# AIRI-Institute/nablaDFT

Measured on NVIDIA H100. Metric: molecules/sec (PaiNN E+F fwd+bwd), higher is better.
Workload: dtype f32

## Files before the change

include/nabla_b200.h:

```cpp
#ifndef NABLA_B200_H
#define NABLA_B200_H

#include <stdint.h>

#ifdef __cplusplus
extern "C" {
#endif

#define NB200_OK 0
#define NB200_EINVAL -1
#define NB200_EUNSUPPORTED -2
#define NB200_ECUDA -3
#define NB200_ECAPACITY -4
#define NB200_ENEIGHBORS -5
#define NB200_ENOEDGES -6

#define NB200_RADIAL_SPK 0
#define NB200_RADIAL_OC 1

int nb200_version(void);
int nb200_last_cuda_error(void);

int nb200_neighbor_build(const float* pos, const int32_t* mol_ptr, int32_t n_mol, int32_t n_atoms,
                         float cutoff, int32_t max_neighbors, int32_t e_cap,
                         int32_t* row_ptr, int32_t* col, int32_t* rev, float* geom,
                         int32_t* deg_scratch, int32_t* status, void* stream);

int nb200_painn_filter(const float* geom, const int32_t* status, int32_t e_stride,
                       const float* w_rbf, const float* b_rbf, int32_t n_layers, int32_t n_rbf,
                       int32_t n_feat, int32_t radial_mode, float cutoff,
                       const float* rbf_offsets, float rbf_coeff, float rbf_xscale,
                       float* W, float* dW, int32_t* sort_scratch, void* stream);

int nb200_painn_msg_fwd(const float* xh, const float* xh_bias, const float* q, const float* mu,
                        const float* W, const float* geom, const int32_t* row_ptr,
                        const int32_t* col, int32_t n_atoms, float* q_out, float* mu_out,
                        void* stream);

int nb200_painn_msg_bwd(const float* xh, const float* xh_bias, const float* mu,
                        const float* W, const float* dW, const float* geom,
                        const int32_t* row_ptr, const int32_t* col, int32_t n_atoms,
                        const float* g_q, const float* g_mu,
                        float* g_xh, float* g_mu_in, float* egrad, void* stream);

int nb200_painn_msg_fwd_ex(const float* xh, const float* xh_bias, const float* q, const float* mu,
                           const void* W, int32_t w_stride, const int32_t* rev, const float* geom,
                           const int32_t* row_ptr, const int32_t* col, int32_t n_atoms, float* q_out,
                           float* mu_out, int32_t bf16, void* stream);
int nb200_painn_msg_bwd_ex(const float* xh, const float* xh_bias, const float* mu, const void* W,
                           const void* dW, int32_t w_stride, const int32_t* rev, const float* geom,
                           const int32_t* row_ptr, const int32_t* col, int32_t n_atoms, const float* g_q,
                           const float* g_mu, float* g_xh, float* g_mu_in, float* egrad, void* gW,
                           const float* seed_atom, int32_t bf16, void* stream);
int nb200_msg_gather_probe(const float* A, const float* B, const float* rec, int32_t rec_stride,
                           const int32_t* rev, const int32_t* row_ptr, const int32_t* col, int32_t n_atoms,
                           int32_t bwd_pattern, float* out, void* stream);

int nb200_edge_forces(const float* egrad, const float* geom, const int32_t* row_ptr,
                      const int32_t* rev, int32_t n_atoms, float* forces, void* stream);

typedef struct nb200_painn_weights {
    int32_t n_layers, n_feat, n_rbf, n_elem;
    int32_t radial_mode, z_offset;
    float cutoff, epsilon;
    float rbf_coeff, rbf_xscale;
    const float* rbf_offsets;
    float energy_shift_per_atom;
    int32_t max_neighbors;
    const float* emb;
    const float* w_rbf;
    const float* b_rbf;
    const float* A1; const float* c1;
    const float* A2; const float* c2;
    const float* U;
    const float* B1; const float* d1;
    const float* B2; const float* d2;
    const float* R1; const float* e1;
    const float* R2; const float* e2;
} nb200_painn_weights;

typedef struct nb200_engine nb200_engine;

int nb200_engine_create(nb200_engine** out);
int nb200_engine_destroy(nb200_engine* eng);
int nb200_engine_set_timing(nb200_engine* eng, int32_t enable);
int nb200_engine_read_timings(nb200_engine* eng, float* ms_per_cat, int32_t* scopes_per_cat, int32_t n_cat);
int nb200_engine_set_gemm_backend(nb200_engine* eng, int32_t backend);
int nb200_engine_set_node_backend(nb200_engine* eng, int32_t backend);
int nb200_gemm_tf32x3(int32_t M, int32_t N, int32_t K, const float* A, int32_t lda, const float* B,
                      int32_t ldb, int32_t trans_b, float* C, int32_t ldc, int32_t accumulate,
                      const float* bias, float* act, void* stream);
int nb200_linear_wgrad(int32_t M, int32_t out, int32_t in, const float* G0, const float* X0, const float* G1,
                       const float* X1, int32_t ldg, int32_t ldx, float* dW, int32_t lddw, float alpha,
                       float* dbias, float bias_alpha, const float* row_scale, int32_t rs_div, void* stream);
int nb200_engine_set_edge_storage(nb200_engine* eng, int32_t bf16);
int64_t nb200_engine_own_launches(nb200_engine* eng);
int64_t nb200_painn_workspace_bytes(const nb200_painn_weights* w, int32_t b_cap, int32_t n_cap,
                                    int32_t e_cap, int32_t with_forces);
int nb200_painn_energy_forces(nb200_engine* eng, const nb200_painn_weights* w,
                              const int32_t* z, const float* pos, const int32_t* mol_ptr,
                              int32_t n_mol, int32_t n_atoms, int32_t e_cap,
                              void* workspace, int64_t workspace_bytes,
                              float* energy, float* forces, int32_t* status, void* stream);
int64_t nb200_painn_train_workspace_bytes(const nb200_painn_weights* w, int32_t b_cap, int32_t n_cap,
                                          int32_t e_cap, int32_t with_force_seed);
int nb200_painn_energy_forces_grads(nb200_engine* eng, const nb200_painn_weights* w,
                                    const int32_t* z, const float* pos, const int32_t* mol_ptr,
                                    int32_t n_mol, int32_t n_atoms, int32_t e_cap,
                                    void* workspace, int64_t workspace_bytes,
                                    const float* energy_seed, const float* force_seed,
                                    const nb200_painn_weights* grads,
                                    float* energy, float* forces, int32_t* status, void* stream);
int nb200_painn_train_forward(nb200_engine* eng, const nb200_painn_weights* w,
                              const int32_t* z, const float* pos, const int32_t* mol_ptr,
                              int32_t n_mol, int32_t n_atoms, int32_t e_cap,
                              void* workspace, int64_t workspace_bytes, int32_t with_force_seed,
                              float* energy, float* forces, int32_t* status, void* stream);
int nb200_painn_train_backward(nb200_engine* eng, const nb200_painn_weights* w,
                               const int32_t* z, const int32_t* mol_ptr,
                               int32_t n_mol, int32_t n_atoms, int32_t e_cap,
                               void* workspace, int64_t workspace_bytes, int32_t with_force_seed,
                               const float* energy_seed, const float* force_seed,
                               const nb200_painn_weights* grads, int32_t* status, void* stream);
int64_t nb200_painn_hvp_workspace_bytes(const nb200_painn_weights* w, int32_t b_cap, int32_t n_cap, int32_t e_cap, int32_t n_dir);
int nb200_painn_hvp(nb200_engine* eng, const nb200_painn_weights* w, const int32_t* z, const float* pos, const int32_t* mol_ptr,
                    int32_t n_mol, int32_t n_atoms, int32_t e_cap, void* workspace, int64_t workspace_bytes,
                    int32_t n_dir, const float* v, float* energy, float* forces, float* hv, int32_t* status, void* stream);

typedef struct nb200_schnet_weights {
    int32_t n_layers, n_feat, n_rbf, n_elem;
    int32_t z_offset;
    float cutoff, rbf_coeff;
    float energy_shift_per_atom;
    const float* rbf_offsets;
    const float* emb;
    const float* w_f1; const float* b_f1;
    const float* W_f2; const float* b_f2;
    const float* I1;
    const float* P1; const float* p1;
    const float* P2; const float* p2;
    const float* R1; const float* e1;
    const float* R2; const float* e2;
} nb200_schnet_weights;

int64_t nb200_schnet_workspace_bytes(const nb200_schnet_weights* w, int32_t b_cap, int32_t n_cap,
                                     int32_t e_cap, int32_t with_forces);
int nb200_schnet_energy_forces(nb200_engine* eng, const nb200_schnet_weights* w,
                               const int32_t* z, const float* pos, const int32_t* mol_ptr,
                               int32_t n_mol, int32_t n_atoms, int32_t e_cap,
                               void* workspace, int64_t workspace_bytes,
                               float* energy, float* forces, int32_t* status, void* stream);

int nb200_schnet_train_count(const nb200_schnet_weights* w, const float* pos, const int32_t* mol_ptr, int32_t n_mol, int32_t n_atoms,
                             int32_t* row_ptr, int32_t* scratch, int64_t* n_edges_host, void* stream);
int64_t nb200_schnet_train_workspace_bytes(const nb200_schnet_weights* w, int32_t n_mol, int32_t n_atoms, int64_t n_edges,
                                           int32_t with_force_seed);
int nb200_schnet_energy_grads(nb200_engine* eng, const nb200_schnet_weights* w, const int32_t* z, const float* pos, const int32_t* mol_ptr,
                              int32_t n_mol, int32_t n_atoms, const int32_t* row_ptr, int64_t n_edges, void* workspace,
                              int64_t workspace_bytes, const float* energy_seed, const float* force_seed,
                              const nb200_schnet_weights* grads, float* energy, void* stream);
int64_t nb200_schnet_hvp_workspace_bytes(const nb200_schnet_weights* w, int32_t n_mol, int32_t n_atoms, int64_t n_edges);
int nb200_schnet_hvp(nb200_engine* eng, const nb200_schnet_weights* w, const int32_t* z, const float* pos, const int32_t* mol_ptr,
                     int32_t n_mol, int32_t n_atoms, const int32_t* row_ptr, int64_t n_edges, void* workspace, int64_t workspace_bytes,
                     int32_t n_dir, const float* v, float* energy, float* forces, float* hv, void* stream);

int nb200_qh_expand_rows(const int32_t* row_ptr, int32_t n_atoms, int32_t* tgt, void* stream);
int nb200_qh_edge_basis(const float* geom, const int32_t* status, int32_t e_cap, double alpha, float cutoff,
                        float sign, const double* logc, int32_t n_rbf, float* rbf, float* sh, void* stream);
int nb200_qh_norm_feats(const float* x, int32_t n_rows, float* f0, void* stream);
int nb200_qh_gate(const float* x, const float* gates, int32_t n_rows, float* y, void* stream);
int nb200_qh_invariants(const float* f, const int32_t* tgt, const int32_t* col, const int32_t* status,
                        int32_t e_cap, int32_t mode, float* out, void* stream);
int nb200_qh_tp_conv(const float* x, const float* sh, const float* w1, const float* w2, const int32_t* row_ptr,
                     const int32_t* col, int32_t n_atoms, int32_t layer0, int32_t add_self, float* out, void* stream);
int nb200_qh_tp_pair(const float* x, const float* w1, const float* w2, const int32_t* tgt, const int32_t* col,
                     const int32_t* status, int32_t p_cap, float* out, void* stream);
int nb200_qh_tp_self(const float* xl, const float* xr, const float* w, const float* res, int32_t n_rows,
                     float* out, void* stream);
int nb200_qh_linear(const float* x, const float* W_l, const float* bias, int32_t n_rows, int32_t c_in,
                    int32_t c_out, int32_t accumulate, float* y, void* stream);
int nb200_dense(int32_t M, int32_t N, int32_t K, const float* A, int32_t lda, const float* B, int32_t ldb,
                int32_t trans_b, float* C, int32_t ldc, int32_t accumulate, const float* bias, float* act,
                int32_t act_kind, void* stream);
int nb200_qh_expand_setup(const int32_t* ins_host, const float* cg_host);
int nb200_qh_expand(const float* x, const float* W, const float* Bw, int32_t bw_stride, int32_t n_rows,
                    float* blocks, void* stream);
int nb200_qh_pair_hidden(const float* A, const float* Bn, const float* bias, const int32_t* tgt,
                         const int32_t* col, const int32_t* status, int32_t p_cap, float* h, void* stream);
int nb200_qh_assemble(const float* diag, const float* offd, const int32_t* z, const int32_t* tgt,
                      const int32_t* col, const int32_t* rev, int32_t n_atoms, int32_t n_pairs,
                      const int32_t* mask_tab, const int32_t* norb_tab, const int32_t* atom_mol,
                      const int32_t* atom_orb_off, const int64_t* mol_h_off, const int32_t* mol_norb,
                      float* H, void* stream);
int nb200_axpy(float* y, const float* x, int64_t n, void* stream);

int64_t nb200_lbfgs_state_bytes(int32_t n_mol, int32_t n_atoms, int32_t memory);
int nb200_lbfgs_step(void* state, int64_t state_bytes, const int32_t* mol_ptr, int32_t n_mol, int32_t n_atoms,
                     int32_t max_atoms_per_mol, int32_t memory, int32_t iteration, double fmax, double maxstep,
                     double damping, double h0, const uint8_t* fixed_mask, double* pos, float* forces,
                     float* pos32_out, int32_t* unconverged_out, int32_t* n_normalizations, void* stream);

int nb200_md_init_momenta(const int32_t* mol_ptr, int32_t n_mol, const double* mass, const double* pos, double kT, uint64_t seed,
                          int64_t noise_step, double* mom, void* stream);
int nb200_md_step(const int32_t* mol_ptr, int32_t n_mol, const double* mass, int32_t phase, int32_t thermostat, double dt, double kT,
                  double gamma, uint64_t seed, int64_t step, double f_scale, double e_scale, double* pos, double* mom, float* pos32,
                  const float* forces, const float* energy, double* log_slot, double* frame_pos, double* frame_mom,
                  const int32_t* status, int32_t* worst, void* stream);

enum {
    NB200_GOC_G_RBF_OFFSET = 0,
    NB200_GOC_G_EMB,
    NB200_GOC_G_CAT_MAIN,
    NB200_GOC_G_CAT_AE,
    NB200_GOC_G_CAT_Q,
    NB200_GOC_G_CAT_A2A,
    NB200_GOC_G_EDGE_EMB,
    NB200_GOC_G_OUT_E0,
    NB200_GOC_G_OUT_E_RES,
    NB200_GOC_G_OUT_ENERGY,
    NB200_GOC_G_OUT_F0,
    NB200_GOC_G_OUT_F_RES,
    NB200_GOC_G_OUT_FORCES,
    NB200_GOC_G_COUNT
};
enum {
    NB200_GOC_I_DENSE_CA = 0,
    NB200_GOC_I_T_BA, NB200_GOC_I_T_RBF , NB200_GOC_I_T_BIL , NB200_GOC_I_T_DOWN ,
    NB200_GOC_I_T_UPCA , NB200_GOC_I_T_UPAC,
    NB200_GOC_I_Q_DB, NB200_GOC_I_Q_RBF, NB200_GOC_I_Q_CBF , NB200_GOC_I_Q_BIL , NB200_GOC_I_Q_DOWN ,
    NB200_GOC_I_Q_UPCA , NB200_GOC_I_Q_UPAC,
    NB200_GOC_I_AE_BA , NB200_GOC_I_AE_RBF , NB200_GOC_I_AE_BIL, NB200_GOC_I_AE_DOWN ,
    NB200_GOC_I_AE_UPCA , NB200_GOC_I_AE_UPAC,
    NB200_GOC_I_EA_BA , NB200_GOC_I_EA_RBF, NB200_GOC_I_EA_BIL, NB200_GOC_I_EA_DOWN , NB200_GOC_I_EA_UP ,
    NB200_GOC_I_AA_BIL , NB200_GOC_I_AA_DOWN , NB200_GOC_I_AA_UP ,
    NB200_GOC_I_BEFORE_SKIP,
    NB200_GOC_I_AFTER_SKIP,
    NB200_GOC_I_AU_RBF , NB200_GOC_I_AU_L0 , NB200_GOC_I_AU_RES ,
    NB200_GOC_I_CONCAT , NB200_GOC_I_RES_M ,
    NB200_GOC_I_COUNT
};
enum {
    NB200_GOC_O_RBF = 0 , NB200_GOC_O_L0 , NB200_GOC_O_RES ,
    NB200_GOC_O_E2 , NB200_GOC_O_F , NB200_GOC_O_RBF_F ,
    NB200_GOC_O_COUNT
};
enum {
    NB200_GOC_S_T_RBF = 0, NB200_GOC_S_Q_RBF, NB200_GOC_S_Q_CBF, NB200_GOC_S_AE_RBF, NB200_GOC_S_EA_RBF, NB200_GOC_S_AU_SUM, NB200_GOC_S_COUNT
};
enum { NB200_GOC_SO_SUM = 0, NB200_GOC_SO_RBF_F, NB200_GOC_SO_COUNT };
enum {
    NB200_GOC_C_A2A = 0,
    NB200_GOC_C_MAIN,
    NB200_GOC_C_AE,
    NB200_GOC_C_Q,
    NB200_GOC_C_TIN,
    NB200_GOC_C_COUNT = 8
};
typedef struct nb200_gemnet_oc_weights {
    int32_t num_blocks;
    int32_t n_elem;
    float cutoff;
    int32_t max_neighbors, max_neighbors_qint, max_neighbors_aeaint;
    const float* w;
    const int64_t* off_host;
    const float* scale_host;
} nb200_gemnet_oc_weights;
int64_t nb200_gemnet_oc_graph_bytes(int32_t n_atoms, int32_t max_atoms_per_mol);
int nb200_gemnet_oc_graph_count(const nb200_gemnet_oc_weights* w, const float* pos, const int32_t* mol_ptr, int32_t n_mol,
                                int32_t n_atoms, int32_t max_atoms_per_mol, void* graph_buf, int64_t graph_bytes,
                                int64_t* counts_host, void* stream);
int64_t nb200_gemnet_oc_workspace_bytes(const nb200_gemnet_oc_weights* w, int32_t n_mol, int32_t n_atoms, const int64_t* counts_host);
int nb200_gemnet_oc_energy_forces(nb200_engine* eng, const nb200_gemnet_oc_weights* w, const int32_t* z, const float* pos,
                                  const int32_t* mol_ptr, int32_t n_mol, int32_t n_atoms, int32_t max_atoms_per_mol,
                                  void* graph_buf, int64_t graph_bytes, const int64_t* counts_host, void* workspace,
                                  int64_t workspace_bytes, float* energy, float* forces, void* stream);
int nb200_gemnet_oc_count_bounds(const nb200_gemnet_oc_weights* w, const int32_t* mol_ptr_host, int32_t n_mol, int64_t* counts_bound_host);
int nb200_gemnet_oc_energy_forces_async(nb200_engine* eng, const nb200_gemnet_oc_weights* w, const int32_t* z, const float* pos,
                                        const int32_t* mol_ptr, int32_t n_mol, int32_t n_atoms, int32_t max_atoms_per_mol,
                                        void* graph_buf, int64_t graph_bytes, const int64_t* counts_bound_host, void* workspace,
                                        int64_t workspace_bytes, float* energy, float* forces, int32_t* status, void* stream);
int64_t nb200_gemnet_oc_train_workspace_bytes(const nb200_gemnet_oc_weights* w, int32_t n_mol, int32_t n_atoms, const int64_t* counts_host);
int nb200_gemnet_oc_energy_forces_grads(nb200_engine* eng, const nb200_gemnet_oc_weights* w, int64_t n_weights, const int32_t* z,
                                        const float* pos, const int32_t* mol_ptr, int32_t n_mol, int32_t n_atoms, int32_t max_atoms_per_mol,
                                        void* graph_buf, int64_t graph_bytes, const int64_t* counts_host, void* workspace,
                                        int64_t workspace_bytes, const float* energy_seed, const float* force_seed, float* grads,
                                        float* energy, float* forces, int64_t* keep_token_host, void* stream);
int nb200_gemnet_oc_backward(nb200_engine* eng, int64_t token, const float* energy_seed, const float* force_seed, void* stream);
int nb200_gemnet_oc_debug_h(const void* workspace, const nb200_gemnet_oc_weights* w, int32_t n_mol, int32_t n_atoms,
                            const int64_t* counts_host, float* h_out, void* stream);

enum {
    NB200_DPP_G_FREQ = 0,
    NB200_DPP_G_ZEROS,
    NB200_DPP_G_NORMS,
    NB200_DPP_G_EMB_TI,
    NB200_DPP_G_EMB_TJ,
    NB200_DPP_G_EMB_RBF_W,
    NB200_DPP_G_EMB_RBF_B,
    NB200_DPP_G_EMB_W3,
    NB200_DPP_G_HEAD_W0, NB200_DPP_G_HEAD_B0,
    NB200_DPP_G_HEAD_W1, NB200_DPP_G_HEAD_B1,
    NB200_DPP_G_HEAD_W2, NB200_DPP_G_HEAD_B2,
    NB200_DPP_G_HEAD_W3, NB200_DPP_G_HEAD_B3,
    NB200_DPP_G_COUNT
};
enum {
    NB200_DPP_I_RBF = 0,
    NB200_DPP_I_SBF,
    NB200_DPP_I_SBF1,
    NB200_DPP_I_SBF2,
    NB200_DPP_I_JI_W, NB200_DPP_I_JI_B, NB200_DPP_I_KJ_W, NB200_DPP_I_KJ_B,
    NB200_DPP_I_DOWN,
    NB200_DPP_I_UP,
    NB200_DPP_I_RES_W,
    NB200_DPP_I_RES_B,
    NB200_DPP_I_LIN_W, NB200_DPP_I_LIN_B,
    NB200_DPP_I_COUNT
};
enum {
    NB200_DPP_O_RBF = 0,
    NB200_DPP_O_UP,
    NB200_DPP_O_LINS_W,
    NB200_DPP_O_LINS_B,
    NB200_DPP_O_LIN,
    NB200_DPP_O_COUNT
};
enum { NB200_DPP_C_EDGES = 0, NB200_DPP_C_TRIPLETS, NB200_DPP_C_COUNT = 4 };
typedef struct nb200_dimenet_weights {
    int32_t num_blocks, node_latent_dim, hidden, int_emb, basis_emb, out_emb, num_spherical, num_radial;
    int32_t num_before_skip, num_after_skip, num_output_layers, envelope_exponent, max_neighbors;
    float cutoff, scale, mean;
    const float* w;
    const int64_t* off_host;
} nb200_dimenet_weights;
int64_t nb200_dimenet_graph_bytes(const nb200_dimenet_weights* w, int32_t n_atoms);
int nb200_dimenet_graph_count(const nb200_dimenet_weights* w, const int32_t* z, const float* pos, const int32_t* mol_ptr, int32_t n_mol,
                              int32_t n_atoms, void* graph_buf, int64_t graph_bytes, int64_t* counts_host, void* stream);
int64_t nb200_dimenet_workspace_bytes(const nb200_dimenet_weights* w, int32_t n_mol, int32_t n_atoms, const int64_t* counts_host);
int nb200_dimenet_energy_forces(nb200_engine* eng, const nb200_dimenet_weights* w, const int32_t* z, const float* pos, const int32_t* mol_ptr,
                                int32_t n_mol, int32_t n_atoms, void* graph_buf, int64_t graph_bytes, const int64_t* counts_host,
                                void* workspace, int64_t workspace_bytes, float* energy, float* forces, float* graph_emb, void* stream);
int nb200_dimenet_debug_sbf_radial(const nb200_dimenet_weights* w, const float* dist, int32_t n, float* rbs, float* drbs, void* stream);

int nb200_phis_n_paths(int32_t order_in1, int32_t order_in2, int32_t order_out, int32_t strict_upper);
int nb200_phis_pair_mixing(const float* x1, const float* x2, const float* coeff, int32_t n_rows, int32_t n_feat,
                           int32_t order_in1, int32_t order_in2, int32_t order_out, float* y, void* stream);
int nb200_phis_self_mixing(const float* x, const float* mixcoeff, const float* keepcoeff, int32_t n_rows, int32_t n_feat,
                           int32_t order_in, int32_t order_out, float* y, void* stream);
int nb200_phis_linear(const float* x, const float* W_l, const float* bias, int32_t n_rows, int32_t c_in, int32_t c_out,
                      int32_t order, float* y, void* stream);

int nb200_phis_swish_self_mixing(const float* x, const float* alpha, const float* beta, const float* mixcoeff, const float* keepcoeff,
                                 int32_t n_rows, int32_t n_feat, float* y, void* stream);
int nb200_phis_linear_ex(const float* x, const float* W_l, const float* bias, int32_t n_rows, int32_t c_in, int32_t c_out, int32_t order,
                         int32_t accumulate, float* y, void* stream);
int nb200_phis_interaction(const float* yi, const float* yj, const float* sh, const float* coeff, const float* wa1, const float* ba1,
                           const float* wa2, const float* ba2, const int32_t* row_ptr, const int32_t* col, int32_t n_atoms, int32_t n_feat,
                           float* y, void* stream);
int nb200_phis_pair_features(const float* fpc, const float* fpn, const float* coeff, const int32_t* row_ptr, const int32_t* col,
                             int32_t n_atoms, int32_t n_feat, float* fii, float* fij, void* stream);
int nb200_phis_overlap_pairs(const float* x, const float* sh, const float* coeff, const float* wa, const int32_t* row_ptr,
                             const int32_t* col, int32_t n_atoms, int32_t n_feat, float* s, void* stream);
int nb200_phis_assemble(const float* Xd, const float* Xo, const float* Wd, const float* bd, int32_t n_col_d, const float* Wo, const float* bo,
                        int32_t n_col_o, int32_t n_feat, const int32_t* atom_el, const int32_t* row_orb, const int32_t* row_m,
                        const int32_t* orb_l, const int32_t* n_rows, const int32_t* ent_range, const int32_t* op_base, const int32_t* ent_col,
                        const int32_t* ent_L, int32_t n_el, int32_t max_ent, const int32_t* tgt, const int32_t* col, const int32_t* rev,
                        int32_t n_atoms, int32_t n_pairs, const int32_t* atom_mol, const int32_t* atom_off, const int64_t* mol_off,
                        const int32_t* mol_norb, int32_t unit_diagonal, float* M, void* stream);

#ifdef __cplusplus
}
#endif
#endif
```

nabladft_b200/_lib.py:

```python
import ctypes
import os
from ctypes import c_double, POINTER, c_float, c_int32, c_int64, c_uint64, c_void_p

_HERE = os.path.dirname(os.path.abspath(__file__))
LIB_PATH = os.path.join(_HERE, "libnabla_b200.so")

NB200_OK = 0
ERRORS = {
    -1: "NB200_EINVAL (bad argument)",
    -2: "NB200_EUNSUPPORTED (configuration outside the compiled fast path)",
    -3: "NB200_ECUDA (CUDA runtime / cuBLAS error)",
    -4: "NB200_ECAPACITY (edge capacity exceeded)",
    -5: "NB200_ENEIGHBORS (an atom has more than max_neighbors neighbours)",
    -6: "NB200_ENOEDGES (an atom has no neighbours)",
}
RADIAL_SPK, RADIAL_OC = 0, 1

_fp = POINTER(c_float)


class PainnWeights(ctypes.Structure):

    _fields_ = [
        ("n_layers", c_int32), ("n_feat", c_int32), ("n_rbf", c_int32), ("n_elem", c_int32),
        ("radial_mode", c_int32), ("z_offset", c_int32),
        ("cutoff", c_float), ("epsilon", c_float),
        ("rbf_coeff", c_float), ("rbf_xscale", c_float),
        ("rbf_offsets", c_void_p),
        ("energy_shift_per_atom", c_float),
        ("max_neighbors", c_int32),
        ("emb", c_void_p), ("w_rbf", c_void_p), ("b_rbf", c_void_p),
        ("A1", c_void_p), ("c1", c_void_p), ("A2", c_void_p), ("c2", c_void_p),
        ("U", c_void_p),
        ("B1", c_void_p), ("d1", c_void_p), ("B2", c_void_p), ("d2", c_void_p),
        ("R1", c_void_p), ("e1", c_void_p), ("R2", c_void_p), ("e2", c_void_p),
    ]


class SchnetWeights(ctypes.Structure):

    _fields_ = [
        ("n_layers", c_int32), ("n_feat", c_int32), ("n_rbf", c_int32), ("n_elem", c_int32),
        ("z_offset", c_int32),
        ("cutoff", c_float), ("rbf_coeff", c_float),
        ("energy_shift_per_atom", c_float),
        ("rbf_offsets", c_void_p),
        ("emb", c_void_p),
        ("w_f1", c_void_p), ("b_f1", c_void_p), ("W_f2", c_void_p), ("b_f2", c_void_p),
        ("I1", c_void_p),
        ("P1", c_void_p), ("p1", c_void_p), ("P2", c_void_p), ("p2", c_void_p),
        ("R1", c_void_p), ("e1", c_void_p), ("R2", c_void_p), ("e2", c_void_p),
    ]


class GemNetOCWeights(ctypes.Structure):

    _fields_ = [("num_blocks", c_int32), ("n_elem", c_int32), ("cutoff", c_float), ("max_neighbors", c_int32), ("max_neighbors_qint", c_int32),
                ("max_neighbors_aeaint", c_int32), ("w", c_void_p), ("off_host", POINTER(c_int64)), ("scale_host", POINTER(c_float))]


class DimeNetWeights(ctypes.Structure):

    _fields_ = [("num_blocks", c_int32), ("node_latent_dim", c_int32), ("hidden", c_int32), ("int_emb", c_int32), ("basis_emb", c_int32),
                ("out_emb", c_int32), ("num_spherical", c_int32), ("num_radial", c_int32), ("num_before_skip", c_int32), ("num_after_skip", c_int32),
                ("num_output_layers", c_int32), ("envelope_exponent", c_int32), ("max_neighbors", c_int32), ("cutoff", c_float), ("scale", c_float),
                ("mean", c_float), ("w", c_void_p), ("off_host", POINTER(c_int64))]


SIGNATURES = {
    "nb200_version": (c_int32, []),
    "nb200_last_cuda_error": (c_int32, []),
    "nb200_neighbor_build": (c_int32, [c_void_p, c_void_p, c_int32, c_int32, c_float, c_int32, c_int32,
                                       c_void_p, c_void_p, c_void_p, c_void_p, c_void_p, c_void_p, c_void_p]),
    "nb200_painn_filter": (c_int32, [c_void_p, c_void_p, c_int32, c_void_p, c_void_p, c_int32, c_int32, c_int32, c_int32,
                                     c_float, c_void_p, c_float, c_float, c_void_p, c_void_p, c_void_p, c_void_p]),
    "nb200_painn_msg_fwd": (c_int32, [c_void_p] * 8 + [c_int32, c_void_p, c_void_p, c_void_p]),
    "nb200_painn_msg_bwd": (c_int32, [c_void_p] * 8 + [c_int32] + [c_void_p] * 6),
    "nb200_edge_forces": (c_int32, [c_void_p, c_void_p, c_void_p, c_void_p, c_int32, c_void_p, c_void_p]),
    "nb200_painn_msg_fwd_ex": (c_int32, [c_void_p] * 5 + [c_int32] + [c_void_p] * 4 + [c_int32] + [c_void_p] * 2 + [c_int32, c_void_p]),
    "nb200_painn_msg_bwd_ex": (c_int32, [c_void_p] * 5 + [c_int32] + [c_void_p] * 4 + [c_int32] + [c_void_p] * 7 + [c_int32, c_void_p]),
    "nb200_msg_gather_probe": (c_int32, [c_void_p] * 3 + [c_int32] + [c_void_p] * 3 + [c_int32, c_int32, c_void_p, c_void_p]),
    "nb200_engine_create": (c_int32, [POINTER(c_void_p)]),
    "nb200_engine_destroy": (c_int32, [c_void_p]),
    "nb200_engine_set_timing": (c_int32, [c_void_p, c_int32]),
    "nb200_engine_read_timings": (c_int32, [c_void_p, c_void_p, c_void_p, c_int32]),
    "nb200_engine_own_launches": (c_int64, [c_void_p]),
    "nb200_engine_set_gemm_backend": (c_int32, [c_void_p, c_int32]),
    "nb200_engine_set_node_backend": (c_int32, [c_void_p, c_int32]),
    "nb200_phis_n_paths": (c_int32, [c_int32, c_int32, c_int32, c_int32]),
    "nb200_phis_pair_mixing": (c_int32, [c_void_p, c_void_p, c_void_p, c_int32, c_int32, c_int32, c_int32, c_int32, c_void_p, c_void_p]),
    "nb200_phis_self_mixing": (c_int32, [c_void_p, c_void_p, c_void_p, c_int32, c_int32, c_int32, c_int32, c_void_p, c_void_p]),
    "nb200_phis_linear": (c_int32, [c_void_p, c_void_p, c_void_p, c_int32, c_int32, c_int32, c_int32, c_void_p, c_void_p]),
    "nb200_phis_swish_self_mixing": (c_int32, [c_void_p] * 5 + [c_int32, c_int32, c_void_p, c_void_p]),
    "nb200_phis_linear_ex": (c_int32, [c_void_p, c_void_p, c_void_p, c_int32, c_int32, c_int32, c_int32, c_int32, c_void_p, c_void_p]),
    "nb200_phis_interaction": (c_int32, [c_void_p] * 10 + [c_int32, c_int32, c_void_p, c_void_p]),
    "nb200_phis_pair_features": (c_int32, [c_void_p] * 5 + [c_int32, c_int32, c_void_p, c_void_p, c_void_p]),
    "nb200_phis_overlap_pairs": (c_int32, [c_void_p] * 6 + [c_int32, c_int32, c_void_p, c_void_p]),
    "nb200_phis_assemble": (c_int32, [c_void_p] * 4 + [c_int32] + [c_void_p] * 2 + [c_int32, c_int32] + [c_void_p] * 9 + [c_int32, c_int32]
                            + [c_void_p] * 3 + [c_int32, c_int32] + [c_void_p] * 4 + [c_int32, c_void_p, c_void_p]),
    "nb200_gemm_tf32x3": (c_int32, [c_int32, c_int32, c_int32, c_void_p, c_int32, c_void_p, c_int32, c_int32, c_void_p, c_int32,
                                    c_int32, c_void_p, c_void_p, c_void_p]),
    "nb200_linear_wgrad": (c_int32, [c_int32, c_int32, c_int32, c_void_p, c_void_p, c_void_p, c_void_p, c_int32, c_int32, c_void_p, c_int32, c_float,
                                     c_void_p, c_float, c_void_p, c_int32, c_void_p]),
    "nb200_qh_expand_rows": (c_int32, [c_void_p, c_int32, c_void_p, c_void_p]),
    "nb200_qh_edge_basis": (c_int32, [c_void_p, c_void_p, c_int32, c_double, c_float, c_float, c_void_p, c_int32, c_void_p, c_void_p, c_void_p]),
    "nb200_qh_norm_feats": (c_int32, [c_void_p, c_int32, c_void_p, c_void_p]),
    "nb200_qh_gate": (c_int32, [c_void_p, c_void_p, c_int32, c_void_p, c_void_p]),
    "nb200_qh_invariants": (c_int32, [c_void_p, c_void_p, c_void_p, c_void_p, c_int32, c_int32, c_void_p, c_void_p]),
    "nb200_qh_tp_conv": (c_int32, [c_void_p] * 6 + [c_int32, c_int32, c_int32, c_void_p, c_void_p]),
    "nb200_qh_tp_pair": (c_int32, [c_void_p] * 6 + [c_int32, c_void_p, c_void_p]),
    "nb200_qh_tp_self": (c_int32, [c_void_p] * 4 + [c_int32, c_void_p, c_void_p]),
    "nb200_qh_linear": (c_int32, [c_void_p, c_void_p, c_void_p, c_int32, c_int32, c_int32, c_int32, c_void_p, c_void_p]),
    "nb200_dense": (c_int32, [c_int32, c_int32, c_int32, c_void_p, c_int32, c_void_p, c_int32, c_int32, c_void_p, c_int32, c_int32,
                              c_void_p, c_void_p, c_int32, c_void_p]),
    "nb200_qh_expand_setup": (c_int32, [c_void_p, c_void_p]),
    "nb200_qh_expand": (c_int32, [c_void_p, c_void_p, c_void_p, c_int32, c_int32, c_void_p, c_void_p]),
    "nb200_qh_pair_hidden": (c_int32, [c_void_p] * 6 + [c_int32, c_void_p, c_void_p]),
    "nb200_qh_assemble": (c_int32, [c_void_p] * 6 + [c_int32, c_int32] + [c_void_p] * 8),
    "nb200_axpy": (c_int32, [c_void_p, c_void_p, c_int64, c_void_p]),
    "nb200_lbfgs_state_bytes": (c_int64, [c_int32, c_int32, c_int32]),
    "nb200_lbfgs_step": (c_int32, [c_void_p, c_int64, c_void_p, c_int32, c_int32, c_int32, c_int32, c_int32, c_double, c_double, c_double,
                                   c_double, c_void_p, c_void_p, c_void_p, c_void_p, c_void_p, c_void_p, c_void_p]),
    "nb200_md_init_momenta": (c_int32, [c_void_p, c_int32, c_void_p, c_void_p, c_double, c_uint64, c_int64, c_void_p, c_void_p]),
    "nb200_md_step": (c_int32, [c_void_p, c_int32, c_void_p, c_int32, c_int32, c_double, c_double, c_double, c_uint64, c_int64, c_double, c_double]
                      + [c_void_p] * 11),
    "nb200_painn_workspace_bytes": (c_int64, [POINTER(PainnWeights), c_int32, c_int32, c_int32, c_int32]),
    "nb200_schnet_workspace_bytes": (c_int64, [POINTER(SchnetWeights), c_int32, c_int32, c_int32, c_int32]),
    "nb200_schnet_energy_forces": (c_int32, [c_void_p, POINTER(SchnetWeights), c_void_p, c_void_p, c_void_p, c_int32, c_int32,
                                             c_int32, c_void_p, c_int64, c_void_p, c_void_p, c_void_p, c_void_p]),
    "nb200_painn_train_workspace_bytes": (c_int64, [POINTER(PainnWeights), c_int32, c_int32, c_int32, c_int32]),
    "nb200_painn_energy_forces_grads": (c_int32, [c_void_p, POINTER(PainnWeights), c_void_p, c_void_p, c_void_p, c_int32, c_int32, c_int32,
                                                  c_void_p, c_int64, c_void_p, c_void_p, POINTER(PainnWeights), c_void_p, c_void_p, c_void_p,
                                                  c_void_p]),
    "nb200_engine_set_edge_storage": (c_int32, [c_void_p, c_int32]),
    "nb200_painn_train_forward": (c_int32, [c_void_p, POINTER(PainnWeights), c_void_p, c_void_p, c_void_p, c_int32, c_int32, c_int32,
                                            c_void_p, c_int64, c_int32, c_void_p, c_void_p, c_void_p, c_void_p]),
    "nb200_painn_train_backward": (c_int32, [c_void_p, POINTER(PainnWeights), c_void_p, c_void_p, c_int32, c_int32, c_int32,
                                             c_void_p, c_int64, c_int32, c_void_p, c_void_p, POINTER(PainnWeights), c_void_p, c_void_p]),
    "nb200_painn_energy_forces": (c_int32, [c_void_p, POINTER(PainnWeights), c_void_p, c_void_p, c_void_p, c_int32, c_int32,
                                            c_int32, c_void_p, c_int64, c_void_p, c_void_p, c_void_p, c_void_p]),
    "nb200_painn_hvp_workspace_bytes": (c_int64, [POINTER(PainnWeights), c_int32, c_int32, c_int32, c_int32]),
    "nb200_painn_hvp": (c_int32, [c_void_p, POINTER(PainnWeights), c_void_p, c_void_p, c_void_p, c_int32, c_int32, c_int32, c_void_p, c_int64,
                                  c_int32, c_void_p, c_void_p, c_void_p, c_void_p, c_void_p, c_void_p]),

    "nb200_gemnet_oc_graph_bytes": (c_int64, [c_int32, c_int32]),
    "nb200_gemnet_oc_graph_count": (c_int32, [POINTER(GemNetOCWeights), c_void_p, c_void_p, c_int32, c_int32, c_int32, c_void_p, c_int64,
                                              POINTER(c_int64), c_void_p]),
    "nb200_gemnet_oc_workspace_bytes": (c_int64, [POINTER(GemNetOCWeights), c_int32, c_int32, POINTER(c_int64)]),
    "nb200_gemnet_oc_energy_forces": (c_int32, [c_void_p, POINTER(GemNetOCWeights), c_void_p, c_void_p, c_void_p, c_int32, c_int32, c_int32,
                                                c_void_p, c_int64, POINTER(c_int64), c_void_p, c_int64, c_void_p, c_void_p, c_void_p]),
    "nb200_gemnet_oc_count_bounds": (c_int32, [POINTER(GemNetOCWeights), POINTER(c_int32), c_int32, POINTER(c_int64)]),
    "nb200_gemnet_oc_energy_forces_async": (c_int32, [c_void_p, POINTER(GemNetOCWeights), c_void_p, c_void_p, c_void_p, c_int32, c_int32, c_int32,
                                                      c_void_p, c_int64, POINTER(c_int64), c_void_p, c_int64, c_void_p, c_void_p, c_void_p, c_void_p]),
    "nb200_gemnet_oc_debug_h": (c_int32, [c_void_p, POINTER(GemNetOCWeights), c_int32, c_int32, POINTER(c_int64), c_void_p, c_void_p]),
    "nb200_schnet_train_count": (c_int32, [POINTER(SchnetWeights), c_void_p, c_void_p, c_int32, c_int32, c_void_p, c_void_p, POINTER(c_int64), c_void_p]),
    "nb200_schnet_train_workspace_bytes": (c_int64, [POINTER(SchnetWeights), c_int32, c_int32, c_int64, c_int32]),
    "nb200_schnet_energy_grads": (c_int32, [c_void_p, POINTER(SchnetWeights), c_void_p, c_void_p, c_void_p, c_int32, c_int32, c_void_p, c_int64, c_void_p,
                                            c_int64, c_void_p, c_void_p, POINTER(SchnetWeights), c_void_p, c_void_p]),
    "nb200_schnet_hvp_workspace_bytes": (c_int64, [POINTER(SchnetWeights), c_int32, c_int32, c_int64]),
    "nb200_schnet_hvp": (c_int32, [c_void_p, POINTER(SchnetWeights), c_void_p, c_void_p, c_void_p, c_int32, c_int32, c_void_p, c_int64, c_void_p,
                                   c_int64, c_int32, c_void_p, c_void_p, c_void_p, c_void_p, c_void_p]),
    "nb200_gemnet_oc_train_workspace_bytes": (c_int64, [POINTER(GemNetOCWeights), c_int32, c_int32, POINTER(c_int64)]),
    "nb200_gemnet_oc_energy_forces_grads": (c_int32, [c_void_p, POINTER(GemNetOCWeights), c_int64, c_void_p, c_void_p, c_void_p, c_int32, c_int32, c_int32,
                                                      c_void_p, c_int64, POINTER(c_int64), c_void_p, c_int64, c_void_p, c_void_p, c_void_p, c_void_p, c_void_p,
                                                      POINTER(c_int64), c_void_p]),
    "nb200_gemnet_oc_backward": (c_int32, [c_void_p, c_int64, c_void_p, c_void_p, c_void_p]),
    "nb200_dimenet_graph_bytes": (c_int64, [POINTER(DimeNetWeights), c_int32]),
    "nb200_dimenet_graph_count": (c_int32, [POINTER(DimeNetWeights), c_void_p, c_void_p, c_void_p, c_int32, c_int32, c_void_p, c_int64,
                                            POINTER(c_int64), c_void_p]),
    "nb200_dimenet_workspace_bytes": (c_int64, [POINTER(DimeNetWeights), c_int32, c_int32, POINTER(c_int64)]),
    "nb200_dimenet_energy_forces": (c_int32, [c_void_p, POINTER(DimeNetWeights), c_void_p, c_void_p, c_void_p, c_int32, c_int32, c_void_p, c_int64,
                                              POINTER(c_int64), c_void_p, c_int64, c_void_p, c_void_p, c_void_p, c_void_p]),
    "nb200_dimenet_debug_sbf_radial": (c_int32, [POINTER(DimeNetWeights), c_void_p, c_int32, c_void_p, c_void_p, c_void_p]),
}

_lib = None


class NablaB200Error(RuntimeError):
    pass


def load():
    global _lib
    if _lib is not None:
        return _lib
    if not os.path.exists(LIB_PATH):
        raise NablaB200Error(
            f"{LIB_PATH} is missing: build it with `python -m nabladft_b200.build` "
            "(nvcc, sm_90a). There is no CPU / eager fallback for this path."
        )
    lib = ctypes.CDLL(LIB_PATH)
    for name, (res, args) in SIGNATURES.items():
        fn = getattr(lib, name)
        fn.restype, fn.argtypes = res, args
    _lib = lib
    return lib


def check(rc: int, what: str):
    if rc != NB200_OK:
        detail = ERRORS.get(rc, f"error {rc}")
        cuda = load().nb200_last_cuda_error() if rc == -3 else 0
        raise NablaB200Error(f"{what} failed: {detail}" + (f" [cudaError {cuda}]" if cuda else ""))


def ptr(t):
    if t is None:
        return None
    assert t.is_contiguous(), "C ABI takes contiguous buffers"
    return c_void_p(t.data_ptr())


def current_stream():
    import torch

    return c_void_p(torch.cuda.current_stream().cuda_stream)
```

nabladft_b200/csrc/painn_fused.cu:

```cuda
#include "painn_node.cuh"

#include "tc_pipe.cuh"

namespace {

constexpr int TILES_PER_LAYER = 22;

enum { T_UV = 0, T_UW, T_B1A, T_B1B, T_B2_0, T_B2_1, T_B2_2, T_A1, T_A2_0, T_A2_1, T_A2_2,
       T_B2T_0, T_B2T_1, T_B2T_2, T_B1AT, T_B1BT, T_UT_0, T_UT_1, T_A2T_0, T_A2T_1, T_A2T_2, T_A1T };

struct TileSrc { const float* p; int ld, row0, k0, trans, rows, kvalid; };

__device__ __forceinline__ TileSrc tile_src(const nb200_painn_weights& w, int idx) {
    const int L = w.n_layers;
    TileSrc s{nullptr, F, 0, 0, 0, 128, 128};
    if (idx >= L * TILES_PER_LAYER) {
        s.p = w.R1; s.ld = F;
        if (idx - L * TILES_PER_LAYER == 0) { s.rows = F / 2; } else { s.trans = 1; s.kvalid = F / 2; }
        return s;
    }
    const int l = idx / TILES_PER_LAYER, t = idx % TILES_PER_LAYER;
    const float* A1 = w.A1 + (size_t)l * F * F;
    const float* A2 = w.A2 + (size_t)l * 3 * F * F;
    const float* U = w.U + (size_t)l * 2 * F * F;
    const float* B1 = w.B1 + (size_t)l * F * 2 * F;
    const float* B2 = w.B2 + (size_t)l * 3 * F * F;
    switch (t) {
        case T_UV: s.p = U; break;
        case T_UW: s.p = U; s.row0 = F; break;
        case T_B1A: s.p = B1; s.ld = 2 * F; break;
        case T_B1B: s.p = B1; s.ld = 2 * F; s.k0 = F; break;
        case T_B2_0: case T_B2_1: case T_B2_2: s.p = B2; s.row0 = (t - T_B2_0) * F; break;
        case T_A1: s.p = A1; break;
        case T_A2_0: case T_A2_1: case T_A2_2: s.p = A2; s.row0 = (t - T_A2_0) * F; break;
        case T_B2T_0: case T_B2T_1: case T_B2T_2: s.p = B2; s.trans = 1; s.k0 = (t - T_B2T_0) * F; break;
        case T_B1AT: s.p = B1; s.ld = 2 * F; s.trans = 1; break;
        case T_B1BT: s.p = B1; s.ld = 2 * F; s.trans = 1; s.row0 = F; break;
        case T_UT_0: case T_UT_1: s.p = U; s.trans = 1; s.k0 = (t - T_UT_0) * F; break;
        case T_A2T_0: case T_A2T_1: case T_A2T_2: s.p = A2; s.trans = 1; s.k0 = (t - T_A2T_0) * F; break;
        default: s.p = A1; s.trans = 1; break;
    }
    return s;
}

__global__ void __launch_bounds__(256) k_prep_painn(nb200_painn_weights w, unsigned char* __restrict__ dst) {
    const int idx = blockIdx.x >> 2, st = blockIdx.x & 3;
    const TileSrc s = tile_src(w, idx);
    unsigned char* tile = dst + (size_t)idx * WTILE_BYTES;
#pragma unroll
    for (int i = 0; i < 4; ++i) {
        const int item = threadIdx.x + 256 * i;
        int kc, r;
        if (!s.trans) { kc = item & 7; r = item >> 3; } else { r = item & 127; kc = item >> 7; }
        const int k = st * 32 + kc * 4;
        float e[4];
#pragma unroll
        for (int j = 0; j < 4; ++j) {
            const bool ok = r < s.rows && k + j < s.kvalid;
            e[j] = !ok ? 0.f : !s.trans ? __ldg(s.p + (size_t)(s.row0 + r) * s.ld + s.k0 + k + j) : __ldg(s.p + (size_t)(s.k0 + k + j) * s.ld + s.row0 + r);
        }
        float4 hi, lo;
        split4(make_float4(e[0], e[1], e[2], e[3]), hi, lo);
        const int kk = 32 * st + 4 * kc;
        float* out_hi = reinterpret_cast<float*>(tile + (size_t)(kk / KSTAGE) * WST_BYTES + (size_t)((kk % KSTAGE) / 4) * WLBO) + r * 4;
        st4(out_hi, hi);
        st4(out_hi + (KSTAGE / 4) * WLBO / 4, lo);
    }
}

struct FwdParams {
    int n_atoms, do_upd, do_mlp, do_ro;
    const unsigned char* wt;
    int tile_upd, tile_mlp, tile_ro;
    const float *q_mid, *mu_mid, *d1, *d2;
    float *VW, *nrm, *dot, *g1pre, *y, *q_next, *mu_next;
    float eps;
    const float *q_mlp_in, *c1;
    float *h1pre, *xh;
    float* ro_pre;
};

template <class L>
__global__ void __launch_bounds__(NTHREADS, CTAS_PER_SM) k_node_fwd(const FwdParams P) {
    constexpr int CW = L::CW;
    extern __shared__ __align__(1024) unsigned char smem[];
    __shared__ Prog prog;
    const int tid = threadIdx.x, warp = tid >> 5, lane = tid & 31;
    if (tid == 0) {
        prog.n = 0;
        if (P.do_upd) {
            for (int x = 0; x < 3; ++x) {
                prog_add(prog, P.tile_upd + T_UV, U_NEWX | U_FIRST | U_LAST);
                prog_add(prog, P.tile_upd + T_UW, U_FIRST | U_LAST | U_XLAST);
            }
            prog_add(prog, P.tile_upd + T_B1A, U_NEWX | U_FIRST | U_LAST | U_XLAST);
            prog_add(prog, P.tile_upd + T_B1B, U_NEWX | U_FIRST | U_LAST | U_XLAST);
            prog_add(prog, P.tile_upd + T_B2_1, U_NEWX | U_FIRST | U_LAST);
            prog_add(prog, P.tile_upd + T_B2_0, U_FIRST | U_LAST);
            prog_add(prog, P.tile_upd + T_B2_2, U_FIRST | U_LAST | U_XLAST);
        }
        if (P.do_mlp) {
            prog_add(prog, P.tile_mlp + T_A1, U_NEWX | U_FIRST | U_LAST | U_XLAST);
            prog_add(prog, P.tile_mlp + T_A2_0, U_NEWX | U_FIRST | U_LAST);
            prog_add(prog, P.tile_mlp + T_A2_1, U_FIRST | U_LAST);
            prog_add(prog, P.tile_mlp + T_A2_2, U_FIRST | U_LAST | U_XLAST);
        }
        if (P.do_ro) prog_add(prog, P.tile_ro, U_NEWX | U_FIRST | U_LAST | U_XLAST);
    }
    Ctx<L> c = setup<L>(smem, tid);

    if (warp >= WARP_ISSUE) {
        role_regs<L>(true);
        run_issuer(c, prog, P.wt);
    } else {
        role_regs<L>(false);
        const int N = P.n_atoms, A0 = blockIdx.x * L::NT;
        const int fl = 32 * (warp & 3) + lane;
        const int n0 = L::CPT * (warp >> 2);
        if (P.do_upd) {
#pragma unroll 1
            for (int x = 0; x < 3; ++x) {
                load_x(c, tid, [&](int r, int kc) { return A0 + r < N ? ldg4(P.mu_mid + (size_t)(A0 + r) * (3 * F) + x * F + 4 * kc) : f4(0.f); });
#pragma unroll 1
                for (int half = 0; half < 2; ++half) {
                    drain(c, warp);
                    epi_chunks(c, warp, [&](int cb, float (&v)[CW]) {
                        float* dst = P.VW + (size_t)(A0 + n0 + CW * cb) * (6 * F) + x * 2 * F + half * F + fl;
#pragma unroll
                        for (int j = 0; j < CW; ++j)
                            if (A0 + n0 + CW * cb + j < N) dst[(size_t)j * (6 * F)] = v[j];
                    });
                }
            }
            work_barrier();
            load_x(c, tid, [&](int r, int kc) { return A0 + r < N ? ldg4(P.q_mid + (size_t)(A0 + r) * F + 4 * kc) : f4(0.f); });
            {
                const int kc = tid & 31, w = tid >> 5;
#pragma unroll 1
                for (int it0 = 0; it0 < L::RPT; it0 += 2) {
                    float4 V[2][3], Wv[2][3];
#pragma unroll
                    for (int b = 0; b < 2; ++b) {
                        const int a = A0 + w + L::NLOAD * (it0 + b);
                        const float* vv = P.VW + (size_t)min(a, N - 1) * (6 * F) + 4 * kc;
#pragma unroll
                        for (int x = 0; x < 3; ++x) { V[b][x] = ld4(vv + x * 2 * F); Wv[b][x] = ld4(vv + x * 2 * F + F); }
                    }
#pragma unroll
                    for (int b = 0; b < 2; ++b) {
                        const int a = A0 + w + L::NLOAD * (it0 + b);
                        if (a < N) {
                            float4 sq = V[b][0] * V[b][0]; fma4(sq, V[b][1], V[b][1]); fma4(sq, V[b][2], V[b][2]);
                            float4 dt = f4(0.f); fma4(dt, V[b][0], Wv[b][0]); fma4(dt, V[b][1], Wv[b][1]); fma4(dt, V[b][2], Wv[b][2]);
                            st4(P.nrm + (size_t)a * F + 4 * kc, make_float4(sqrtf(sq.x + P.eps), sqrtf(sq.y + P.eps), sqrtf(sq.z + P.eps), sqrtf(sq.w + P.eps)));
                            st4(P.dot + (size_t)a * F + 4 * kc, dt);
                        }
                    }
                }
            }
            work_barrier();
            load_x(c, tid, [&](int r, int kc) { return A0 + r < N ? ld4(P.nrm + (size_t)(A0 + r) * F + 4 * kc) : f4(0.f); });
            drain(c, warp);
            {
                drain(c, warp, 1);
                const float b = __ldg(P.d1 + fl);
                const XPut xp(c, fl);
                epi_chunks(c, warp, [&](int cb, float (&v)[CW]) {
#pragma unroll
                    for (int j = 0; j < CW; ++j) xp.put(n0 + CW * cb + j, A0 + n0 + CW * cb + j < N ? siluf_(v[j] + b) : 0.f);
                });
                xp.done(c);
                epi_chunks(c, warp, [&](int cb, float (&v)[CW]) {
                    float* g = P.g1pre + (size_t)(A0 + n0 + CW * cb) * F + fl;
#pragma unroll
                    for (int j = 0; j < CW; ++j)
                        if (A0 + n0 + CW * cb + j < N) g[(size_t)j * F] = v[j] + b;
                });
            }
            {
                drain(c, warp);
                const float b = __ldg(P.d2 + F + fl);
#pragma unroll 1
                for (int cb = 0; cb < L::CPT / 8; ++cb) {
                    float v8[8];
                    stage_ld(c, warp, 8 * cb, v8);
                    float tw[8][3], tm[8][3];
#pragma unroll
                    for (int jj = 0; jj < 8; ++jj) {
                        const int a = min(A0 + n0 + 8 * cb + jj, N - 1);
                        const float* vw = P.VW + (size_t)a * (6 * F) + F + fl;
                        const float* mm = P.mu_mid + (size_t)a * (3 * F) + fl;
#pragma unroll
                        for (int x = 0; x < 3; ++x) { tw[jj][x] = vw[x * 2 * F]; tm[jj][x] = __ldg(mm + x * F); }
                    }
#pragma unroll
                    for (int jj = 0; jj < 8; ++jj) {
                        const int a = A0 + n0 + 8 * cb + jj;
                        if (a < N) {
                            const float y1 = v8[jj] + b;
                            P.y[(size_t)a * (3 * F) + F + fl] = y1;
                            float* mo = P.mu_next + (size_t)a * (3 * F) + fl;
#pragma unroll
                            for (int x = 0; x < 3; ++x) mo[x * F] = fmaf(y1, tw[jj][x], tm[jj][x]);
                        }
                    }
                }
            }
            {
                drain(c, warp);
                const float b = __ldg(P.d2 + fl);
                epi_chunks(c, warp, [&](int cb, float (&v)[CW]) {
                    float t[CW];
#pragma unroll
                    for (int j = 0; j < CW; ++j) t[j] = __ldg(P.q_mid + (size_t)min(A0 + n0 + CW * cb + j, N - 1) * F + fl);
#pragma unroll
                    for (int j = 0; j < CW; ++j) {
                        const int a = A0 + n0 + CW * cb + j;
                        if (a < N) {
                            const float y0 = v[j] + b;
                            P.y[(size_t)a * (3 * F) + fl] = y0;
                            P.q_next[(size_t)a * F + fl] = t[j] + y0;
                        }
                    }
                });
            }
            {
                drain(c, warp);
                const float b = __ldg(P.d2 + 2 * F + fl);
                const XPut xp(c, fl);
                epi_chunks(c, warp, [&](int cb, float (&v)[CW]) {
                    float tq[CW], td[CW];
#pragma unroll
                    for (int j = 0; j < CW; ++j) {
                        const size_t a = (size_t)min(A0 + n0 + CW * cb + j, N - 1);
                        tq[j] = P.q_next[a * F + fl];
                        td[j] = P.dot[a * F + fl];
                    }
#pragma unroll
                    for (int j = 0; j < CW; ++j) {
                        const int a = A0 + n0 + CW * cb + j;
                        float qn = 0.f;
                        if (a < N) {
                            qn = fmaf(v[j] + b, td[j], tq[j]);
                            P.q_next[(size_t)a * F + fl] = qn;
                        }
                        xp.put(n0 + CW * cb + j, qn);
                    }
                });
                xp.done(c);
                epi_chunks(c, warp, [&](int cb, float (&v)[CW]) {
#pragma unroll
                    for (int j = 0; j < CW; ++j)
                        if (A0 + n0 + CW * cb + j < N) P.y[(size_t)(A0 + n0 + CW * cb + j) * (3 * F) + 2 * F + fl] = v[j] + b;
                });
            }
        } else {
            load_x(c, tid, [&](int r, int kc) { return A0 + r < N ? ldg4(P.q_mlp_in + (size_t)(A0 + r) * F + 4 * kc) : f4(0.f); });
        }
        if (P.do_mlp) {
            {
                drain(c, warp);
                const float b = __ldg(P.c1 + fl);
                const XPut xp(c, fl);
                epi_chunks(c, warp, [&](int cb, float (&v)[CW]) {
#pragma unroll
                    for (int j = 0; j < CW; ++j) xp.put(n0 + CW * cb + j, siluf_(v[j] + b));
                });
                xp.done(c);
                epi_chunks(c, warp, [&](int cb, float (&v)[CW]) {
#pragma unroll
                    for (int j = 0; j < CW; ++j)
                        if (A0 + n0 + CW * cb + j < N) P.h1pre[(size_t)(A0 + n0 + CW * cb + j) * F + fl] = v[j] + b;
                });
            }
#pragma unroll 1
            for (int ct = 0; ct < 3; ++ct) {
                drain(c, warp);
                epi_chunks(c, warp, [&](int cb, float (&v)[CW]) {
                    float* dst = P.xh + (size_t)(A0 + n0 + CW * cb) * (3 * F) + ct * F + fl;
#pragma unroll
                    for (int j = 0; j < CW; ++j)
                        if (A0 + n0 + CW * cb + j < N) dst[(size_t)j * (3 * F)] = v[j];
                });
            }
        }
        if (P.do_ro) {
            drain(c, warp);
            epi_chunks(c, warp, [&](int cb, float (&v)[CW]) {
                if (fl < F / 2) {
                    float* dst = P.ro_pre + (size_t)(A0 + n0 + CW * cb) * (F / 2) + fl;
#pragma unroll
                    for (int j = 0; j < CW; ++j)
                        if (A0 + n0 + CW * cb + j < N) dst[(size_t)j * (F / 2)] = v[j];
                }
            });
        }
    }
}

struct BwdParams {
    int n_atoms, do_mlp, do_ro, do_upd;
    const unsigned char* wt;
    int tile_mlp, tile_ro, tile_upd;
    float *gq_a, *gq_b, *cur, *gn, *gdot;
    const float *g_xh, *h1pre, *dot;
    const float *ro_pre, *R2;
    const float *y, *VW, *nrm, *g1pre;
};

template <class L>
__global__ void __launch_bounds__(NTHREADS, CTAS_PER_SM) k_node_bwd(const BwdParams P) {
    constexpr int CW = L::CW;
    extern __shared__ __align__(1024) unsigned char smem[];
    __shared__ Prog prog;
    const int tid = threadIdx.x, warp = tid >> 5, lane = tid & 31;
    if (tid == 0) {
        prog.n = 0;
        if (P.do_mlp) {
            prog_add(prog, P.tile_mlp + T_A2T_0, U_NEWX | U_FIRST | U_XLAST);
            prog_add(prog, P.tile_mlp + T_A2T_1, U_NEWX | U_XLAST);
            prog_add(prog, P.tile_mlp + T_A2T_2, U_NEWX | U_XLAST | U_LAST);
            prog_add(prog, P.tile_mlp + T_A1T, U_NEWX | U_FIRST | U_LAST | U_XLAST);
        } else if (P.do_ro) {
            prog_add(prog, P.tile_ro, U_NEWX | U_FIRST | U_LAST | U_XLAST);
        }
        if (P.do_upd) {
            prog_add(prog, P.tile_upd + T_B2T_0, U_NEWX | U_FIRST | U_XLAST);
            prog_add(prog, P.tile_upd + T_B2T_1, U_NEWX | U_XLAST);
            prog_add(prog, P.tile_upd + T_B2T_2, U_NEWX | U_XLAST | U_LAST);
            prog_add(prog, P.tile_upd + T_B1AT, U_NEWX | U_FIRST | U_LAST);
            prog_add(prog, P.tile_upd + T_B1BT, U_FIRST | U_LAST | U_XLAST);
            for (int x = 0; x < 3; ++x) {
                prog_add(prog, P.tile_upd + T_UT_0, U_NEWX | U_FIRST | U_XLAST);
                prog_add(prog, P.tile_upd + T_UT_1, U_NEWX | U_XLAST | U_LAST);
            }
        }
    }
    Ctx<L> c = setup<L>(smem, tid);

    if (warp >= WARP_ISSUE) {
        role_regs<L>(true);
        run_issuer(c, prog, P.wt);
    } else {
        role_regs<L>(false);
        const int N = P.n_atoms, A0 = blockIdx.x * L::NT;
        const int fl = 32 * (warp & 3) + lane;
        const int n0 = L::CPT * (warp >> 2);
        if (P.do_mlp) {
#pragma unroll 1
            for (int ck = 0; ck < 3; ++ck)
                load_x(c, tid, [&](int r, int kc) { return A0 + r < N ? ldg4(P.g_xh + (size_t)(A0 + r) * (3 * F) + ck * F + 4 * kc) : f4(0.f); });
            drain(c, warp);
            const XPut xp(c, fl);
            epi_chunks(c, warp, [&](int cb, float (&v)[CW]) {
                float t[CW];
#pragma unroll
                for (int j = 0; j < CW; ++j) t[j] = __ldg(P.h1pre + (size_t)min(A0 + n0 + CW * cb + j, N - 1) * F + fl);
#pragma unroll
                for (int j = 0; j < CW; ++j) xp.put(n0 + CW * cb + j, A0 + n0 + CW * cb + j < N ? v[j] * dsiluf_(t[j]) : 0.f);
            });
            xp.done(c);
        } else if (P.do_ro) {
            load_x(c, tid, [&](int r, int kc) {
                if (A0 + r >= N || kc >= F / 8) return f4(0.f);
                const float4 p = ldg4(P.ro_pre + (size_t)(A0 + r) * (F / 2) + 4 * kc), w2 = ldg4(P.R2 + 4 * kc);
                return make_float4(w2.x * dsiluf_(p.x), w2.y * dsiluf_(p.y), w2.z * dsiluf_(p.z), w2.w * dsiluf_(p.w));
            });
        }
        if (P.do_mlp || P.do_ro) {
            drain(c, warp);
            epi_chunks(c, warp, [&](int cb, float (&v)[CW]) {
                float t[CW], ty[CW];
#pragma unroll
                for (int j = 0; j < CW; ++j) {
                    const size_t a = (size_t)min(A0 + n0 + CW * cb + j, N - 1);
                    t[j] = P.do_mlp ? P.gq_a[a * F + fl] : 0.f;
                    ty[j] = P.do_upd ? __ldg(P.y + a * (3 * F) + 2 * F + fl) : 0.f;
                }
#pragma unroll
                for (int j = 0; j < CW; ++j) {
                    const int a = A0 + n0 + CW * cb + j;
                    if (a < N) {
                        const float g = t[j] + v[j];
                        P.gq_b[(size_t)a * F + fl] = g;
                        if (P.do_upd) P.gdot[(size_t)a * F + fl] = g * ty[j];
                    }
                }
            });
        }
        if (P.do_upd) {
            work_barrier();
            load_x(c, tid, [&](int r, int kc) { return A0 + r < N ? ld4(P.gq_b + (size_t)(A0 + r) * F + 4 * kc) : f4(0.f); });
            load_x(c, tid, [&](int r, int kc) {
                if (A0 + r >= N) return f4(0.f);
                const float* vw = P.VW + (size_t)(A0 + r) * (6 * F) + F + 4 * kc;
                const float* gm = P.cur + (size_t)(A0 + r) * (3 * F) + 4 * kc;
                float4 sacc = f4(0.f);
#pragma unroll
                for (int x = 0; x < 3; ++x) fma4(sacc, ld4(gm + x * F), ldg4(vw + x * 2 * F));
                return sacc;
            });
            load_x(c, tid, [&](int r, int kc) {
                return A0 + r < N ? ld4(P.gq_b + (size_t)(A0 + r) * F + 4 * kc) * ldg4(P.dot + (size_t)(A0 + r) * F + 4 * kc) : f4(0.f);
            });
            drain(c, warp);
            const XPut xp(c, fl);
            epi_chunks(c, warp, [&](int cb, float (&v)[CW]) {
                float t[CW];
#pragma unroll
                for (int j = 0; j < CW; ++j) t[j] = __ldg(P.g1pre + (size_t)min(A0 + n0 + CW * cb + j, N - 1) * F + fl);
#pragma unroll
                for (int j = 0; j < CW; ++j) xp.put(n0 + CW * cb + j, A0 + n0 + CW * cb + j < N ? v[j] * dsiluf_(t[j]) : 0.f);
            });
            xp.done(c);
            {
                drain(c, warp);
                epi_chunks(c, warp, [&](int cb, float (&v)[CW]) {
                    float t[CW];
#pragma unroll
                    for (int j = 0; j < CW; ++j) t[j] = P.gq_b[(size_t)min(A0 + n0 + CW * cb + j, N - 1) * F + fl];
#pragma unroll
                    for (int j = 0; j < CW; ++j)
                        if (A0 + n0 + CW * cb + j < N) P.gq_a[(size_t)(A0 + n0 + CW * cb + j) * F + fl] = t[j] + v[j];
                });
            }
            {
                drain(c, warp);
                epi_chunks(c, warp, [&](int cb, float (&v)[CW]) {
                    float t[CW];
#pragma unroll
                    for (int j = 0; j < CW; ++j) t[j] = __ldg(P.nrm + (size_t)min(A0 + n0 + CW * cb + j, N - 1) * F + fl);
#pragma unroll
                    for (int j = 0; j < CW; ++j)
                        if (A0 + n0 + CW * cb + j < N) P.gn[(size_t)(A0 + n0 + CW * cb + j) * F + fl] = v[j] / t[j];
                });
            }
            work_barrier();
#pragma unroll 1
            for (int x = 0; x < 3; ++x) {
                load_x(c, tid, [&](int r, int kc) {
                    if (A0 + r >= N) return f4(0.f);
                    const size_t a = (size_t)(A0 + r);
                    float4 o = ld4(P.gdot + a * F + 4 * kc) * ldg4(P.VW + a * (6 * F) + x * 2 * F + F + 4 * kc);
                    fma4(o, ld4(P.gn + a * F + 4 * kc), ldg4(P.VW + a * (6 * F) + x * 2 * F + 4 * kc));
                    return o;
                });
                load_x(c, tid, [&](int r, int kc) {
                    if (A0 + r >= N) return f4(0.f);
                    const size_t a = (size_t)(A0 + r);
                    float4 o = ld4(P.cur + a * (3 * F) + x * F + 4 * kc) * ldg4(P.y + a * (3 * F) + F + 4 * kc);
                    fma4(o, ld4(P.gdot + a * F + 4 * kc), ldg4(P.VW + a * (6 * F) + x * 2 * F + 4 * kc));
                    return o;
                });
                drain(c, warp);
                epi_chunks(c, warp, [&](int cb, float (&v)[CW]) {
                    float t[CW];
#pragma unroll
                    for (int j = 0; j < CW; ++j) t[j] = P.cur[(size_t)min(A0 + n0 + CW * cb + j, N - 1) * (3 * F) + x * F + fl];
#pragma unroll
                    for (int j = 0; j < CW; ++j)
                        if (A0 + n0 + CW * cb + j < N) P.cur[(size_t)(A0 + n0 + CW * cb + j) * (3 * F) + x * F + fl] = t[j] + v[j];
                });
            }
        }
    }
}

using Node64 = Layout<false, 64>;
using Node80 = Layout<false, 80>;

bool wide_tiles(int n_atoms) {
    const int sm = nb_sm_count();
    const int waves64 = ((n_atoms + Node64::NT - 1) / Node64::NT + sm - 1) / sm, waves80 = ((n_atoms + Node80::NT - 1) / Node80::NT + sm - 1) / sm;
    return waves80 < waves64;
}

template <class L, class Params>
int launch_tiles(void (*kernel)(Params), const Params& P, int n_atoms, cudaStream_t s) {
    static std::atomic<bool> attr[NB_MAX_DEVICES];
    int dev = 0;
    cudaGetDevice(&dev);
    const bool cached = dev >= 0 && dev < NB_MAX_DEVICES;
    if (!cached || !attr[dev].load(std::memory_order_relaxed)) {
        if (cudaFuncSetAttribute(kernel, cudaFuncAttributeMaxDynamicSharedMemorySize, L::SMEM_TOTAL) != cudaSuccess) { nb_check_launch(); return NB200_ECUDA; }
        if (cached) attr[dev].store(true, std::memory_order_relaxed);
    }
    kernel<<<(n_atoms + L::NT - 1) / L::NT, NTHREADS, L::SMEM_TOTAL, s>>>(P);
    return nb_check_launch();
}

}

int64_t nb_fused_wtile_bytes(int n_layers) { return (int64_t)(n_layers * TILES_PER_LAYER + 2) * WTILE_BYTES; }

int nb_fused_prep(const nb200_painn_weights* w, void* wtiles, cudaStream_t s) {
    const int n_tiles = w->n_layers * TILES_PER_LAYER + 2;
    k_prep_painn<<<n_tiles * 4, 256, 0, s>>>(*w, static_cast<unsigned char*>(wtiles));
    return nb_check_launch();
}

int nb_fused_node_fwd(const NbFusedFwd& a, cudaStream_t s) {
    FwdParams P{};
    P.n_atoms = a.n_atoms; P.do_upd = a.layer_upd >= 0; P.do_mlp = a.layer_mlp >= 0; P.do_ro = a.readout;
    P.wt = static_cast<const unsigned char*>(a.wtiles);
    P.tile_upd = a.layer_upd * TILES_PER_LAYER; P.tile_mlp = a.layer_mlp * TILES_PER_LAYER; P.tile_ro = a.n_layers * TILES_PER_LAYER;
    P.q_mid = a.q_mid; P.mu_mid = a.mu_mid; P.d1 = a.d1; P.d2 = a.d2; P.VW = a.VW; P.nrm = a.nrm; P.dot = a.dot; P.g1pre = a.g1pre; P.y = a.y;
    P.q_next = a.q_next; P.mu_next = a.mu_next; P.eps = a.eps; P.q_mlp_in = a.q_mlp_in; P.c1 = a.c1; P.h1pre = a.h1pre; P.xh = a.xh;
    P.ro_pre = a.ro_pre;
    if (a.n_atoms <= 0) return NB200_OK;
    return wide_tiles(a.n_atoms) ? launch_tiles<Node80>(k_node_fwd<Node80>, P, a.n_atoms, s) : launch_tiles<Node64>(k_node_fwd<Node64>, P, a.n_atoms, s);
}

int nb_fused_node_bwd(const NbFusedBwd& a, cudaStream_t s) {
    BwdParams P{};
    P.n_atoms = a.n_atoms; P.do_mlp = a.layer_mlp >= 0; P.do_ro = a.readout; P.do_upd = a.layer_upd >= 0;
    P.wt = static_cast<const unsigned char*>(a.wtiles);
    P.tile_mlp = a.layer_mlp * TILES_PER_LAYER; P.tile_ro = a.n_layers * TILES_PER_LAYER + 1; P.tile_upd = a.layer_upd * TILES_PER_LAYER;
    P.gq_a = a.gq_a; P.gq_b = a.gq_b; P.cur = a.cur; P.gn = a.gn; P.gdot = a.gdot; P.dot = a.dot; P.g_xh = a.g_xh; P.h1pre = a.h1pre; P.ro_pre = a.ro_pre; P.R2 = a.R2;
    P.y = a.y; P.VW = a.VW; P.nrm = a.nrm; P.g1pre = a.g1pre;
    if (a.n_atoms <= 0) return NB200_OK;
    return wide_tiles(a.n_atoms) ? launch_tiles<Node80>(k_node_bwd<Node80>, P, a.n_atoms, s) : launch_tiles<Node64>(k_node_bwd<Node64>, P, a.n_atoms, s);
}
```

nabladft_b200/csrc/tc_pipe.cuh:

```cuda
#pragma once
#include "common.cuh"
#include "wgmma.cuh"

namespace {


constexpr int F = NB_F;
constexpr int KSTAGE = 32, W_STAGES = 3, NWORK = 8, CTAS_PER_SM = 1;
constexpr int WLBO = 128 * 16;
constexpr int WST_BYTES = 2 * (KSTAGE / 4) * WLBO;
constexpr int STAGES_PER_TILE = 128 / KSTAGE;
constexpr int WTILE_BYTES = STAGES_PER_TILE * WST_BYTES;
template <bool TWO_GROUPS, int NT_ = 64>
struct Layout {
    static constexpr bool two_groups = TWO_GROUPS;
    static constexpr int NT = NT_;
    static constexpr int NEPI = TWO_GROUPS ? NWORK / 2 : NWORK, NLOAD = TWO_GROUPS ? NWORK / 2 : NWORK;
    static constexpr int CPT = NT / (NEPI / 4);
    static constexpr int CW = CPT % 16 == 0 ? 16 : 8;
    static constexpr int RPT = NT / NLOAD;
    static constexpr int XLBO = NT * 16 + 16;
    static constexpr int XLBOF = XLBO / 4;
    static constexpr int X_BYTES = 32 * XLBO;
    static constexpr int SROW = NT + 4;
    static constexpr int STAGE_BYTES = 128 * SROW * 4;
    static constexpr int SMEM_BARS = 2 * X_BYTES + W_STAGES * WST_BYTES + STAGE_BYTES;
    static constexpr int SMEM_TOTAL = SMEM_BARS + 256;
    static constexpr int WORK_REGS = NT == 64 ? 0 : 88, MMA_REGS = NT == 64 ? 0 : 168;
    static_assert(NT == 64 || NT == 80, "the wgmma N of the pipeline (wgmma_tf32_nt)");
    static_assert(SMEM_TOTAL <= 227 * 1024, "shared memory of one CTA");
    static_assert((XLBO / 16) % 2 == 1 && XLBO % 128 == 16, "X padding: 8 chunk writers of a row / 32 feature writers of a column hit distinct banks");
    static_assert((SROW / 4) % 2 == 1, "staging padding: the 16-byte reads of 8 consecutive feature rows hit 8 bank groups");
    static_assert(CPT % CW == 0 && CW % 4 == 0, "epilogue chunks");
    static_assert(WORK_REGS + MMA_REGS == 0 || WORK_REGS + MMA_REGS == 2 * 128, "the register split must hand over exactly what it takes");
};
using OneGroup = Layout<false>;
using TwoGroups = Layout<true>;
constexpr int WARP_ISSUE = NWORK;
constexpr int NTHREADS = 32 * (NWORK + 8);
static_assert(NWORK % 4 == 0, "the MMA warpgroups must start on a warpgroup boundary");
static_assert(NWORK * 32 == NTHREADS / 2, "role_regs: the worker and MMA warpgroups hold the same number of threads");

template <class L>
__device__ __forceinline__ void role_regs(bool mma) {
    if constexpr (L::MMA_REGS > 0) {
        if (mma) asm volatile("setmaxnreg.inc.sync.aligned.u32 %0;" ::"n"(L::MMA_REGS));
        else asm volatile("setmaxnreg.dec.sync.aligned.u32 %0;" ::"n"(L::WORK_REGS));
    }
}

template <int NT>
__device__ __forceinline__ void wgmma_tf32_nt(float (&d)[NT / 2], uint64_t da, uint64_t db) {
    if constexpr (NT == 64) wgmma_tf32_n64(d, da, db);
    else wgmma_tf32_n80(d, da, db);
}
enum { U_NEWX = 1, U_FIRST = 2, U_LAST = 4, U_XLAST = 8 };

struct Prog {
    int n;
    uint16_t tile[24];
    uint8_t flag[24];
};

__device__ __forceinline__ void work_barrier() { asm volatile("bar.sync 1, %0;" ::"n"(32 * NWORK) : "memory"); }
__device__ __forceinline__ float4 ld4(const float* p) { return *reinterpret_cast<const float4*>(p); }

template <class L>
struct Ctx {
    float *x_hi, *x_lo;
    unsigned char* ring;
    float* stage;
    uint64_t *full, *empty, *x_ready, *x_free, *acc_full, *stage_free;
    uint64_t *x_ready2, *x_free2;
    int xg = 0;
    int o = 0;
};

template <class L, class FlagFn, class TileFn>
__device__ __forceinline__ void run_issuer_t(Ctx<L>& c, int n_units, FlagFn flags_of, TileFn tile_of, const unsigned char* wt, int spt = STAGES_PER_TILE) {
    constexpr int NT = L::NT, XLBO = L::XLBO;
    const int wl = ((threadIdx.x >> 5) - WARP_ISSUE) & 3, h = ((threadIdx.x >> 5) - WARP_ISSUE) >> 2, lane = threadIdx.x & 31;
    float corr[NT / 2], main0[NT / 2], main1[NT / 2];
    const uint32_t x_hi0 = s_u32(c.x_hi), x_lo0 = s_u32(c.x_lo);
    const int n_q = n_units * spt;
    const bool leader = threadIdx.x == 32 * WARP_ISSUE;
    int q = 0, pending = -1;
    auto release = [&](uint64_t* bar) { if (lane == 0) mbar_arrive(bar); };
    auto copy = [&](int qq) {
        if (!leader || qq >= n_q) return;
        const int slot = qq % W_STAGES;
        mbar_expect_tx(c.full + slot, WST_BYTES);
        bulk_g2s(c.ring + slot * WST_BYTES, wt + (size_t)tile_of(qq / spt) * WTILE_BYTES + (size_t)(qq % spt) * WST_BYTES, WST_BYTES, c.full + slot);
    };
    auto free_stage = [&](int pq) {
        const int slot = pq % W_STAGES;
        release(c.empty + slot);
        if (leader) { mbar_wait(c.empty + slot, (uint32_t)((pq / W_STAGES) & 1)); copy(pq + W_STAGES); }
    };
    for (int qq = 0; qq < W_STAGES; ++qq) copy(qq);
#pragma unroll 1
    for (int u = 0; u < n_units; ++u) {
        const int fl = flags_of(u);
        const bool newx = (fl & U_NEWX) != 0;
        if (newx) { mbar_wait(c.x_ready, (uint32_t)(c.xg & 1)); ++c.xg; }
        if (fl & U_FIRST) {
#pragma unroll
            for (int i = 0; i < NT / 2; ++i) { corr[i] = 0.f; main0[i] = 0.f; main1[i] = 0.f; }
        }
#pragma unroll 1
        for (int st = 0; st < spt; ++st, ++q) {
            const int slot = q % W_STAGES;
            if (L::two_groups && newx && st == STAGES_PER_TILE / 2)
                mbar_wait(c.x_ready2, (uint32_t)((c.xg - 1) & 1));
            mbar_wait(c.full + slot, (uint32_t)((q / W_STAGES) & 1));
            const uint32_t wh = s_u32(c.ring + slot * WST_BYTES), wlo = wh + (KSTAGE / 4) * WLBO;
            const uint32_t xoff = (uint32_t)(st * (KSTAGE / 4) * XLBO);
            wgmma_fence();
#pragma unroll
            for (int ks = 0; ks < KSTAGE / 8; ++ks) {
                const uint64_t dxh = gmma_desc(x_hi0 + xoff + 2 * ks * XLBO, XLBO, 128), dxl = gmma_desc(x_lo0 + xoff + 2 * ks * XLBO, XLBO, 128);
                const uint64_t dwh = gmma_desc(wh + 2 * ks * WLBO + h * 1024, WLBO, 128), dwl = gmma_desc(wlo + 2 * ks * WLBO + h * 1024, WLBO, 128);
                wgmma_tf32_nt<NT>(corr, dwl, dxh);
                wgmma_tf32_nt<NT>(corr, dwh, dxl);
                if (ks & 1) wgmma_tf32_nt<NT>(main1, dwh, dxh);
                else wgmma_tf32_nt<NT>(main0, dwh, dxh);
            }
            wgmma_commit();
            wgmma_wait<1>();
            if (pending >= 0) free_stage(pending);
            pending = q;
            if (L::two_groups && (fl & U_XLAST) && st == STAGES_PER_TILE / 2 - 1) {
                wgmma_wait<0>();
                free_stage(pending); pending = -1;
                release(c.x_free);
            }
        }
        wgmma_wait<0>();
        if (pending >= 0) { free_stage(pending); pending = -1; }
        if (fl & U_XLAST) {
            if (!L::two_groups) release(c.x_free);
            else { if (spt < STAGES_PER_TILE / 2) release(c.x_free); release(c.x_free2); }
        }
        if (fl & U_LAST) {
            if (c.o > 0) mbar_wait(c.stage_free, (uint32_t)((c.o - 1) & 1));
            const int f = 64 * h + 16 * wl + (lane >> 2);
#pragma unroll
            for (int j = 0; j < NT / 8; ++j) {
                const int n = 8 * j + 2 * (lane & 3);
                *reinterpret_cast<float2*>(c.stage + f * L::SROW + n) = make_float2(corr[4 * j] + (main0[4 * j] + main1[4 * j]), corr[4 * j + 1] + (main0[4 * j + 1] + main1[4 * j + 1]));
                *reinterpret_cast<float2*>(c.stage + (f + 8) * L::SROW + n) = make_float2(corr[4 * j + 2] + (main0[4 * j + 2] + main1[4 * j + 2]), corr[4 * j + 3] + (main0[4 * j + 3] + main1[4 * j + 3]));
            }
            mbar_arrive(c.acc_full);
            ++c.o;
        }
    }
}
template <class L>
__device__ __forceinline__ void run_issuer(Ctx<L>& c, const Prog& prog, const unsigned char* wt) {
    run_issuer_t(c, prog.n, [&](int u) { return (int)prog.flag[u]; }, [&](int u) { return (int)prog.tile[u]; }, wt);
}

template <class L, class Fn>
__device__ __forceinline__ void load_x(Ctx<L>& c, int wtid, Fn f) {
    constexpr int NLOAD = L::NLOAD, NT = L::NT, XLBOF = L::XLBOF;
    if constexpr (L::two_groups) {
        const int lane = wtid & 31, wrp = wtid >> 5, half = wrp >= NLOAD / 2 ? 1 : 0, w8 = wrp - half * (NLOAD / 2);
        const int kc = (lane & 15) + 16 * half, rsub = lane >> 4;
        constexpr int ITEMS = (NT * 16) / (32 * (NLOAD / 2));
        static_assert(ITEMS * 32 * (NLOAD / 2) == NT * 16 && ITEMS <= 16, "load_x two-group mapping");
        float4 t[ITEMS];
#pragma unroll
        for (int it = 0; it < ITEMS; ++it) t[it] = f(2 * (w8 + (NLOAD / 2) * it) + rsub, kc);
        if (c.xg > 0) mbar_wait(half ? c.x_free2 : c.x_free, (uint32_t)((c.xg - 1) & 1));
#pragma unroll
        for (int it = 0; it < ITEMS; ++it) {
            const int r = 2 * (w8 + (NLOAD / 2) * it) + rsub;
            float4 hi, lo;
            split4(t[it], hi, lo);
            st4(c.x_hi + kc * XLBOF + r * 4, hi);
            st4(c.x_lo + kc * XLBOF + r * 4, lo);
        }
        fence_proxy_async();
        mbar_arrive(half ? c.x_ready2 : c.x_ready);
        ++c.xg;
        return;
    }
    constexpr int RB = L::RPT % 8 == 0 ? 8 : L::RPT / 2;
    static_assert(L::RPT % RB == 0, "load_x one-group mapping");
    const int kc = wtid & 31, w = wtid >> 5;
#pragma unroll 1
    for (int h = 0; h < L::RPT / RB; ++h) {
        float4 t[RB];
#pragma unroll
        for (int it = 0; it < RB; ++it) t[it] = f(w + NLOAD * (RB * h + it), kc);
        if (c.xg > 0) mbar_wait(c.x_free, (uint32_t)((c.xg - 1) & 1));
#pragma unroll
        for (int it = 0; it < RB; ++it) {
            const int r = w + NLOAD * (RB * h + it);
            float4 hi, lo;
            split4(t[it], hi, lo);
            st4(c.x_hi + kc * XLBOF + r * 4, hi);
            st4(c.x_lo + kc * XLBOF + r * 4, lo);
        }
    }
    fence_proxy_async();
    mbar_arrive(c.x_ready);
    ++c.xg;
}

template <class L>
struct XPut {
    float *hi, *lo;
    bool second;
    __device__ __forceinline__ XPut(const Ctx<L>& c, int k) {
        second = L::two_groups && k >= 64;
        if (c.xg > 0) mbar_wait(second ? c.x_free2 : c.x_free, (uint32_t)((c.xg - 1) & 1));
        hi = c.x_hi + (k >> 2) * L::XLBOF + (k & 3);
        lo = c.x_lo + (k >> 2) * L::XLBOF + (k & 3);
    }
    __device__ __forceinline__ void put(int n, float v) const {
        float h, l;
        split_tf32(v, h, l);
        hi[n * 4] = h;
        lo[n * 4] = l;
    }
    __device__ __forceinline__ void done(Ctx<L>& c) const {
        fence_proxy_async();
        mbar_arrive(second ? c.x_ready2 : c.x_ready);
        ++c.xg;
    }
};

template <class L>
__device__ __forceinline__ void drain(Ctx<L>& c, int warp, int add_stage = 0) {
    float* mine = c.stage + (32 * (warp & 3) + (threadIdx.x & 31)) * L::SROW + (warp >> 2) * L::CPT;
    if (add_stage) {
        float4 keep[L::CPT / 4];
#pragma unroll
        for (int i = 0; i < L::CPT / 4; ++i) keep[i] = reinterpret_cast<const float4*>(mine)[i];
        if (c.o > 0) mbar_arrive(c.stage_free);
        mbar_wait(c.acc_full, (uint32_t)(c.o & 1));
#pragma unroll
        for (int i = 0; i < L::CPT / 4; ++i) reinterpret_cast<float4*>(mine)[i] = reinterpret_cast<const float4*>(mine)[i] + keep[i];
    } else {
        if (c.o > 0) mbar_arrive(c.stage_free);
        mbar_wait(c.acc_full, (uint32_t)(c.o & 1));
    }
    ++c.o;
}

template <class L, int W>
__device__ __forceinline__ void stage_ld(const Ctx<L>& c, int warp, int col, float (&v)[W]) {
    const float4* src = reinterpret_cast<const float4*>(c.stage + (32 * (warp & 3) + (threadIdx.x & 31)) * L::SROW + (warp >> 2) * L::CPT + col);
#pragma unroll
    for (int i = 0; i < W / 4; ++i) {
        const float4 t = src[i];
        v[4 * i] = t.x; v[4 * i + 1] = t.y; v[4 * i + 2] = t.z; v[4 * i + 3] = t.w;
    }
}

__device__ __forceinline__ void prog_add(Prog& p, int tile, int flags) {
    p.tile[p.n] = (uint16_t)tile;
    p.flag[p.n] = (uint8_t)flags;
    ++p.n;
}

template <class L>
__device__ __forceinline__ Ctx<L> setup(unsigned char* smem, int tid) {
    Ctx<L> c;
    c.x_hi = reinterpret_cast<float*>(smem);
    c.x_lo = reinterpret_cast<float*>(smem + L::X_BYTES);
    c.ring = smem + 2 * L::X_BYTES;
    c.stage = reinterpret_cast<float*>(smem + 2 * L::X_BYTES + W_STAGES * WST_BYTES);
    uint64_t* bars = reinterpret_cast<uint64_t*>(smem + L::SMEM_BARS);
    c.full = bars; c.empty = bars + W_STAGES; c.x_ready = bars + 2 * W_STAGES; c.x_free = c.x_ready + 1; c.acc_full = c.x_ready + 2;
    c.stage_free = c.x_ready + 3; c.x_ready2 = c.x_ready + 4; c.x_free2 = c.x_ready + 5;
    if (tid == 0) {
        for (int s = 0; s < W_STAGES; ++s) { mbar_init(c.full + s, 1); mbar_init(c.empty + s, 8); }
        mbar_init(c.x_ready, L::two_groups ? 16 * L::NLOAD : 32 * L::NLOAD);
        mbar_init(c.x_free, 8);
        if (L::two_groups) {
            mbar_init(c.x_ready2, 16 * L::NLOAD);
            mbar_init(c.x_free2, 8);
        }
        mbar_init(c.acc_full, 256);
        mbar_init(c.stage_free, 32 * L::NEPI);
        asm volatile("fence.mbarrier_init.release.cluster;" ::: "memory");
    }
    __syncthreads();
    return c;
}

template <class L, class Body>
__device__ __forceinline__ void epi_chunks(const Ctx<L>& c, int warp, Body body) {
#pragma unroll 1
    for (int cb = 0; cb < L::CPT / L::CW; ++cb) {
        float v[L::CW];
        stage_ld(c, warp, L::CW * cb, v);
        body(cb, v);
    }
}


}
```

Before: 71650.

## Overlap node-kernel epilogues with next X loads and add stall probe

```diff
diff --git a/include/nabla_b200.h b/include/nabla_b200.h
--- a/include/nabla_b200.h
+++ b/include/nabla_b200.h
@@ -55,6 +55,7 @@
 int nb200_msg_gather_probe(const float* A, const float* B, const float* rec, int32_t rec_stride,
                            const int32_t* rev, const int32_t* row_ptr, const int32_t* col, int32_t n_atoms,
                            int32_t bwd_pattern, float* out, void* stream);
+int nb200_node_stall_probe(int64_t* prof, int32_t max_ctas);
 
 int nb200_edge_forces(const float* egrad, const float* geom, const int32_t* row_ptr,
                       const int32_t* rev, int32_t n_atoms, float* forces, void* stream);
diff --git a/nabladft_b200/_lib.py b/nabladft_b200/_lib.py
--- a/nabladft_b200/_lib.py
+++ b/nabladft_b200/_lib.py
@@ -80,6 +80,7 @@
     "nb200_painn_msg_fwd_ex": (c_int32, [c_void_p] * 5 + [c_int32] + [c_void_p] * 4 + [c_int32] + [c_void_p] * 2 + [c_int32, c_void_p]),
     "nb200_painn_msg_bwd_ex": (c_int32, [c_void_p] * 5 + [c_int32] + [c_void_p] * 4 + [c_int32] + [c_void_p] * 7 + [c_int32, c_void_p]),
     "nb200_msg_gather_probe": (c_int32, [c_void_p] * 3 + [c_int32] + [c_void_p] * 3 + [c_int32, c_int32, c_void_p, c_void_p]),
+    "nb200_node_stall_probe": (c_int32, [c_void_p, c_int32]),
     "nb200_engine_create": (c_int32, [POINTER(c_void_p)]),
     "nb200_engine_destroy": (c_int32, [c_void_p]),
     "nb200_engine_set_timing": (c_int32, [c_void_p, c_int32]),
diff --git a/nabladft_b200/csrc/painn_fused.cu b/nabladft_b200/csrc/painn_fused.cu
--- a/nabladft_b200/csrc/painn_fused.cu
+++ b/nabladft_b200/csrc/painn_fused.cu
@@ -78,7 +78,13 @@
     const float *q_mlp_in, *c1;
     float *h1pre, *xh;
     float* ro_pre;
+    long long* prof; int prof_ctas;
 };
+
+template <class Params>
+__device__ __forceinline__ long long* prof_row(const Params& P) {
+    return P.prof && (int)blockIdx.x < P.prof_ctas ? P.prof + (size_t)blockIdx.x * PR_ROW : nullptr;
+}
 
 template <class L>
 __global__ void __launch_bounds__(NTHREADS, CTAS_PER_SM) k_node_fwd(const FwdParams P) {
@@ -112,55 +118,54 @@
     if (warp >= WARP_ISSUE) {
         role_regs<L>(true);
         run_issuer(c, prog, P.wt);
+        if (tid == 32 * WARP_ISSUE) probe_store(c, prof_row(P), PR_FULL, PR_XFREE);
     } else {
         role_regs<L>(false);
         const int N = P.n_atoms, A0 = blockIdx.x * L::NT;
         const int fl = 32 * (warp & 3) + lane;
         const int n0 = L::CPT * (warp >> 2);
+        const long long t_run = pclock<L>();
         if (P.do_upd) {
+            auto mu_x = [&](int x) {
+                return [&, x](int r, int kc) { return A0 + r < N ? ldg4(P.mu_mid + (size_t)(A0 + r) * (3 * F) + x * F + 4 * kc) : f4(0.f); };
+            };
+            auto vw_epi = [&](int x, int half) {
+                epi_chunks(c, warp, [&](int cb, float (&v)[CW]) {
+                    float* dst = P.VW + (size_t)(A0 + n0 + CW * cb) * (6 * F) + x * 2 * F + half * F + fl;
+#pragma unroll
+                    for (int j = 0; j < CW; ++j)
+                        if (A0 + n0 + CW * cb + j < N) dst[(size_t)j * (6 * F)] = v[j];
+                });
+            };
+            load_x(c, tid, mu_x(0));
 #pragma unroll 1
             for (int x = 0; x < 3; ++x) {
-                load_x(c, tid, [&](int r, int kc) { return A0 + r < N ? ldg4(P.mu_mid + (size_t)(A0 + r) * (3 * F) + x * F + 4 * kc) : f4(0.f); });
-#pragma unroll 1
-                for (int half = 0; half < 2; ++half) {
-                    drain(c, warp);
-                    epi_chunks(c, warp, [&](int cb, float (&v)[CW]) {
-                        float* dst = P.VW + (size_t)(A0 + n0 + CW * cb) * (6 * F) + x * 2 * F + half * F + fl;
-#pragma unroll
-                        for (int j = 0; j < CW; ++j)
-                            if (A0 + n0 + CW * cb + j < N) dst[(size_t)j * (6 * F)] = v[j];
-                    });
-                }
-            }
-            work_barrier();
-            load_x(c, tid, [&](int r, int kc) { return A0 + r < N ? ldg4(P.q_mid + (size_t)(A0 + r) * F + 4 * kc) : f4(0.f); });
-            {
-                const int kc = tid & 31, w = tid >> 5;
-#pragma unroll 1
-                for (int it0 = 0; it0 < L::RPT; it0 += 2) {
-                    float4 V[2][3], Wv[2][3];
-#pragma unroll
-                    for (int b = 0; b < 2; ++b) {
-                        const int a = A0 + w + L::NLOAD * (it0 + b);
-                        const float* vv = P.VW + (size_t)min(a, N - 1) * (6 * F) + 4 * kc;
-#pragma unroll
-                        for (int x = 0; x < 3; ++x) { V[b][x] = ld4(vv + x * 2 * F); Wv[b][x] = ld4(vv + x * 2 * F + F); }
-                    }
-#pragma unroll
-                    for (int b = 0; b < 2; ++b) {
-                        const int a = A0 + w + L::NLOAD * (it0 + b);
-                        if (a < N) {
-                            float4 sq = V[b][0] * V[b][0]; fma4(sq, V[b][1], V[b][1]); fma4(sq, V[b][2], V[b][2]);
-                            float4 dt = f4(0.f); fma4(dt, V[b][0], Wv[b][0]); fma4(dt, V[b][1], Wv[b][1]); fma4(dt, V[b][2], Wv[b][2]);
-                            st4(P.nrm + (size_t)a * F + 4 * kc, make_float4(sqrtf(sq.x + P.eps), sqrtf(sq.y + P.eps), sqrtf(sq.z + P.eps), sqrtf(sq.w + P.eps)));
-                            st4(P.dot + (size_t)a * F + 4 * kc, dt);
-                        }
-                    }
-                }
-            }
-            work_barrier();
-            load_x(c, tid, [&](int r, int kc) { return A0 + r < N ? ld4(P.nrm + (size_t)(A0 + r) * F + 4 * kc) : f4(0.f); });
-            drain(c, warp);
+                drain(c, warp);
+                vw_epi(x, 0);
+                stage_release(c);
+                if (x < 2) load_x(c, tid, mu_x(x + 1));
+                else load_x(c, tid, [&](int r, int kc) { return A0 + r < N ? ldg4(P.q_mid + (size_t)(A0 + r) * F + 4 * kc) : f4(0.f); });
+                drain(c, warp, 0, true);
+                vw_epi(x, 1);
+            }
+            stage_release(c);
+            work_barrier(c);
+            load_x(c, tid, [&](int r, int kc) {
+                const int a = A0 + r;
+                if (a >= N) return f4(0.f);
+                const float* vv = P.VW + (size_t)a * (6 * F) + 4 * kc;
+                float4 V[3], Wv[3];
+#pragma unroll
+                for (int x = 0; x < 3; ++x) { V[x] = ld4(vv + x * 2 * F); Wv[x] = ld4(vv + x * 2 * F + F); }
+                float4 sq = V[0] * V[0]; fma4(sq, V[1], V[1]); fma4(sq, V[2], V[2]);
+                float4 dt = f4(0.f); fma4(dt, V[0], Wv[0]); fma4(dt, V[1], Wv[1]); fma4(dt, V[2], Wv[2]);
+                const float4 nr = make_float4(sqrtf(sq.x + P.eps), sqrtf(sq.y + P.eps), sqrtf(sq.z + P.eps), sqrtf(sq.w + P.eps));
+                st4(P.nrm + (size_t)a * F + 4 * kc, nr);
+                st4(P.dot + (size_t)a * F + 4 * kc, dt);
+                return nr;
+            });
+            work_barrier(c);
+            drain(c, warp, 0, true);
             {
                 drain(c, warp, 1);
                 const float b = __ldg(P.d1 + fl);
@@ -179,6 +184,7 @@
             }
             {
                 drain(c, warp);
+                const long long t0 = pclock<L>();
                 const float b = __ldg(P.d2 + F + fl);
 #pragma unroll 1
                 for (int cb = 0; cb < L::CPT / 8; ++cb) {
@@ -205,6 +211,7 @@
                         }
                     }
                 }
+                pspan(c, PR_EPI, t0);
             }
             {
                 drain(c, warp);
@@ -295,6 +302,8 @@
                 }
             });
         }
+        pspan(c, PR_WORKER, t_run);
+        if (tid == 0) probe_store(c, prof_row(P), PR_XFREE, NPROF);
     }
 }
 
@@ -306,6 +315,7 @@
     const float *g_xh, *h1pre, *dot;
     const float *ro_pre, *R2;
     const float *y, *VW, *nrm, *g1pre;
+    long long* prof; int prof_ctas;
 };
 
 template <class L>
@@ -341,15 +351,17 @@
     if (warp >= WARP_ISSUE) {
         role_regs<L>(true);
         run_issuer(c, prog, P.wt);
+        if (tid == 32 * WARP_ISSUE) probe_store(c, prof_row(P), PR_FULL, PR_XFREE);
     } else {
         role_regs<L>(false);
         const int N = P.n_atoms, A0 = blockIdx.x * L::NT;
         const int fl = 32 * (warp & 3) + lane;
         const int n0 = L::CPT * (warp >> 2);
+        const long long t_run = pclock<L>();
         if (P.do_mlp) {
 #pragma unroll 1
             for (int ck = 0; ck < 3; ++ck)
-                load_x(c, tid, [&](int r, int kc) { return A0 + r < N ? ldg4(P.g_xh + (size_t)(A0 + r) * (3 * F) + ck * F + 4 * kc) : f4(0.f); });
+                load_x<L::RPT>(c, tid, [&](int r, int kc) { return A0 + r < N ? ldg4(P.g_xh + (size_t)(A0 + r) * (3 * F) + ck * F + 4 * kc) : f4(0.f); });
             drain(c, warp);
             const XPut xp(c, fl);
             epi_chunks(c, warp, [&](int cb, float (&v)[CW]) {
@@ -369,28 +381,39 @@
         }
         if (P.do_mlp || P.do_ro) {
             drain(c, warp);
-            epi_chunks(c, warp, [&](int cb, float (&v)[CW]) {
-                float t[CW], ty[CW];
-#pragma unroll
-                for (int j = 0; j < CW; ++j) {
-                    const size_t a = (size_t)min(A0 + n0 + CW * cb + j, N - 1);
-                    t[j] = P.do_mlp ? P.gq_a[a * F + fl] : 0.f;
-                    ty[j] = P.do_upd ? __ldg(P.y + a * (3 * F) + 2 * F + fl) : 0.f;
-                }
-#pragma unroll
-                for (int j = 0; j < CW; ++j) {
-                    const int a = A0 + n0 + CW * cb + j;
-                    if (a < N) {
+            auto gqb_epi = [&](auto put) {
+                epi_chunks(c, warp, [&](int cb, float (&v)[CW]) {
+                    float t[CW], ty[CW];
+#pragma unroll
+                    for (int j = 0; j < CW; ++j) {
+                        const size_t a = (size_t)min(A0 + n0 + CW * cb + j, N - 1);
+                        t[j] = P.do_mlp ? P.gq_a[a * F + fl] : 0.f;
+                        ty[j] = P.do_upd ? __ldg(P.y + a * (3 * F) + 2 * F + fl) : 0.f;
+                    }
+#pragma unroll
+                    for (int j = 0; j < CW; ++j) {
+                        const int a = A0 + n0 + CW * cb + j;
                         const float g = t[j] + v[j];
-                        P.gq_b[(size_t)a * F + fl] = g;
-                        if (P.do_upd) P.gdot[(size_t)a * F + fl] = g * ty[j];
-                    }
-                }
-            });
+                        put(n0 + CW * cb + j, a < N ? g : 0.f);
+                        if (a < N) {
+                            P.gq_b[(size_t)a * F + fl] = g;
+                            if (P.do_upd) P.gdot[(size_t)a * F + fl] = g * ty[j];
+                        }
+                    }
+                });
+            };
+            if (P.do_upd) {
+                const XPut xp(c, fl);
+                gqb_epi([&](int n, float g) { xp.put(n, g); });
+                xp.done(c);
+            } else {
+                gqb_epi([](int, float) {});
+            }
+            stage_release(c);
         }
         if (P.do_upd) {
-            work_barrier();
-            load_x(c, tid, [&](int r, int kc) { return A0 + r < N ? ld4(P.gq_b + (size_t)(A0 + r) * F + 4 * kc) : f4(0.f); });
+            if (!P.do_mlp && !P.do_ro)
+                load_x(c, tid, [&](int r, int kc) { return A0 + r < N ? ld4(P.gq_b + (size_t)(A0 + r) * F + 4 * kc) : f4(0.f); });
             load_x(c, tid, [&](int r, int kc) {
                 if (A0 + r >= N) return f4(0.f);
                 const float* vw = P.VW + (size_t)(A0 + r) * (6 * F) + F + 4 * kc;
@@ -400,24 +423,27 @@
                 for (int x = 0; x < 3; ++x) fma4(sacc, ld4(gm + x * F), ldg4(vw + x * 2 * F));
                 return sacc;
             });
+            work_barrier(c);
             load_x(c, tid, [&](int r, int kc) {
                 return A0 + r < N ? ld4(P.gq_b + (size_t)(A0 + r) * F + 4 * kc) * ldg4(P.dot + (size_t)(A0 + r) * F + 4 * kc) : f4(0.f);
             });
-            drain(c, warp);
-            const XPut xp(c, fl);
-            epi_chunks(c, warp, [&](int cb, float (&v)[CW]) {
-                float t[CW];
-#pragma unroll
-                for (int j = 0; j < CW; ++j) t[j] = __ldg(P.g1pre + (size_t)min(A0 + n0 + CW * cb + j, N - 1) * F + fl);
-#pragma unroll
-                for (int j = 0; j < CW; ++j) xp.put(n0 + CW * cb + j, A0 + n0 + CW * cb + j < N ? v[j] * dsiluf_(t[j]) : 0.f);
-            });
-            xp.done(c);
-            {
-                drain(c, warp);
+            drain(c, warp, 0, P.do_mlp || P.do_ro);
+            {
+                const XPut xp(c, fl);
                 epi_chunks(c, warp, [&](int cb, float (&v)[CW]) {
                     float t[CW];
 #pragma unroll
+                    for (int j = 0; j < CW; ++j) t[j] = __ldg(P.g1pre + (size_t)min(A0 + n0 + CW * cb + j, N - 1) * F + fl);
+#pragma unroll
+                    for (int j = 0; j < CW; ++j) xp.put(n0 + CW * cb + j, A0 + n0 + CW * cb + j < N ? v[j] * dsiluf_(t[j]) : 0.f);
+                });
+                xp.done(c);
+            }
+            {
+                drain(c, warp);
+                epi_chunks(c, warp, [&](int cb, float (&v)[CW]) {
+                    float t[CW];
+#pragma unroll
                     for (int j = 0; j < CW; ++j) t[j] = P.gq_b[(size_t)min(A0 + n0 + CW * cb + j, N - 1) * F + fl];
 #pragma unroll
                     for (int j = 0; j < CW; ++j)
@@ -426,25 +452,55 @@
             }
             {
                 drain(c, warp);
+                const XPut xp(c, fl);
+                epi_chunks(c, warp, [&](int cb, float (&v)[CW]) {
+                    constexpr int H = CW / 2;
+#pragma unroll
+                    for (int h = 0; h < 2; ++h) {
+                        float t[H], gd[H], wv[H], vv[H];
+#pragma unroll
+                        for (int i = 0; i < H; ++i) {
+                            const size_t a = (size_t)min(A0 + n0 + CW * cb + H * h + i, N - 1);
+                            t[i] = __ldg(P.nrm + a * F + fl);
+                            gd[i] = P.gdot[a * F + fl];
+                            wv[i] = __ldg(P.VW + a * (6 * F) + F + fl);
+                            vv[i] = __ldg(P.VW + a * (6 * F) + fl);
+                        }
+#pragma unroll
+                        for (int i = 0; i < H; ++i) {
+                            const int j = H * h + i, a = A0 + n0 + CW * cb + j;
+                            const float sn = v[j] / t[i];
+                            xp.put(n0 + CW * cb + j, a < N ? fmaf(sn, vv[i], gd[i] * wv[i]) : 0.f);
+                            if (a < N) P.gn[(size_t)a * F + fl] = sn;
+                        }
+                    }
+                });
+                xp.done(c);
+                stage_release(c);
+            }
+            work_barrier(c);
+            auto cur_epi = [&](int x) {
+                drain(c, warp, 0, true);
                 epi_chunks(c, warp, [&](int cb, float (&v)[CW]) {
                     float t[CW];
 #pragma unroll
-                    for (int j = 0; j < CW; ++j) t[j] = __ldg(P.nrm + (size_t)min(A0 + n0 + CW * cb + j, N - 1) * F + fl);
-#pragma unroll
-                    for (int j = 0; j < CW; ++j)
-                        if (A0 + n0 + CW * cb + j < N) P.gn[(size_t)(A0 + n0 + CW * cb + j) * F + fl] = v[j] / t[j];
-                });
-            }
-            work_barrier();
+                    for (int j = 0; j < CW; ++j) t[j] = P.cur[(size_t)min(A0 + n0 + CW * cb + j, N - 1) * (3 * F) + x * F + fl];
+#pragma unroll
+                    for (int j = 0; j < CW; ++j)
+                        if (A0 + n0 + CW * cb + j < N) P.cur[(size_t)(A0 + n0 + CW * cb + j) * (3 * F) + x * F + fl] = t[j] + v[j];
+                });
+                stage_release(c);
+            };
 #pragma unroll 1
             for (int x = 0; x < 3; ++x) {
-                load_x(c, tid, [&](int r, int kc) {
-                    if (A0 + r >= N) return f4(0.f);
-                    const size_t a = (size_t)(A0 + r);
-                    float4 o = ld4(P.gdot + a * F + 4 * kc) * ldg4(P.VW + a * (6 * F) + x * 2 * F + F + 4 * kc);
-                    fma4(o, ld4(P.gn + a * F + 4 * kc), ldg4(P.VW + a * (6 * F) + x * 2 * F + 4 * kc));
-                    return o;
-                });
+                if (x > 0)
+                    load_x(c, tid, [&](int r, int kc) {
+                        if (A0 + r >= N) return f4(0.f);
+                        const size_t a = (size_t)(A0 + r);
+                        float4 o = ld4(P.gdot + a * F + 4 * kc) * ldg4(P.VW + a * (6 * F) + x * 2 * F + F + 4 * kc);
+                        fma4(o, ld4(P.gn + a * F + 4 * kc), ldg4(P.VW + a * (6 * F) + x * 2 * F + 4 * kc));
+                        return o;
+                    });
                 load_x(c, tid, [&](int r, int kc) {
                     if (A0 + r >= N) return f4(0.f);
                     const size_t a = (size_t)(A0 + r);
@@ -452,22 +508,22 @@
                     fma4(o, ld4(P.gdot + a * F + 4 * kc), ldg4(P.VW + a * (6 * F) + x * 2 * F + 4 * kc));
                     return o;
                 });
-                drain(c, warp);
-                epi_chunks(c, warp, [&](int cb, float (&v)[CW]) {
-                    float t[CW];
-#pragma unroll
-                    for (int j = 0; j < CW; ++j) t[j] = P.cur[(size_t)min(A0 + n0 + CW * cb + j, N - 1) * (3 * F) + x * F + fl];
-#pragma unroll
-                    for (int j = 0; j < CW; ++j)
-                        if (A0 + n0 + CW * cb + j < N) P.cur[(size_t)(A0 + n0 + CW * cb + j) * (3 * F) + x * F + fl] = t[j] + v[j];
-                });
-            }
-        }
+                if (x > 0) cur_epi(x - 1);
+            }
+            cur_epi(2);
+        }
+        pspan(c, PR_WORKER, t_run);
+        if (tid == 0) probe_store(c, prof_row(P), PR_XFREE, NPROF);
     }
 }
 
 using Node64 = Layout<false, 64>;
 using Node80 = Layout<false, 80>;
+using Node64P = Layout<false, 64, true>;
+using Node80P = Layout<false, 80, true>;
+
+long long* g_prof = nullptr;
+int g_prof_ctas = 0;
 
 bool wide_tiles(int n_atoms) {
     const int sm = nb_sm_count();
@@ -508,7 +564,12 @@
     P.q_next = a.q_next; P.mu_next = a.mu_next; P.eps = a.eps; P.q_mlp_in = a.q_mlp_in; P.c1 = a.c1; P.h1pre = a.h1pre; P.xh = a.xh;
     P.ro_pre = a.ro_pre;
     if (a.n_atoms <= 0) return NB200_OK;
-    return wide_tiles(a.n_atoms) ? launch_tiles<Node80>(k_node_fwd<Node80>, P, a.n_atoms, s) : launch_tiles<Node64>(k_node_fwd<Node64>, P, a.n_atoms, s);
+    const bool wide = wide_tiles(a.n_atoms);
+    if (g_prof) {
+        P.prof = g_prof; P.prof_ctas = g_prof_ctas;
+        return wide ? launch_tiles<Node80P>(k_node_fwd<Node80P>, P, a.n_atoms, s) : launch_tiles<Node64P>(k_node_fwd<Node64P>, P, a.n_atoms, s);
+    }
+    return wide ? launch_tiles<Node80>(k_node_fwd<Node80>, P, a.n_atoms, s) : launch_tiles<Node64>(k_node_fwd<Node64>, P, a.n_atoms, s);
 }
 
 int nb_fused_node_bwd(const NbFusedBwd& a, cudaStream_t s) {
@@ -519,5 +580,17 @@
     P.gq_a = a.gq_a; P.gq_b = a.gq_b; P.cur = a.cur; P.gn = a.gn; P.gdot = a.gdot; P.dot = a.dot; P.g_xh = a.g_xh; P.h1pre = a.h1pre; P.ro_pre = a.ro_pre; P.R2 = a.R2;
     P.y = a.y; P.VW = a.VW; P.nrm = a.nrm; P.g1pre = a.g1pre;
     if (a.n_atoms <= 0) return NB200_OK;
-    return wide_tiles(a.n_atoms) ? launch_tiles<Node80>(k_node_bwd<Node80>, P, a.n_atoms, s) : launch_tiles<Node64>(k_node_bwd<Node64>, P, a.n_atoms, s);
-}
+    const bool wide = wide_tiles(a.n_atoms);
+    if (g_prof) {
+        P.prof = g_prof + (size_t)g_prof_ctas * PR_ROW; P.prof_ctas = g_prof_ctas;
+        return wide ? launch_tiles<Node80P>(k_node_bwd<Node80P>, P, a.n_atoms, s) : launch_tiles<Node64P>(k_node_bwd<Node64P>, P, a.n_atoms, s);
+    }
+    return wide ? launch_tiles<Node80>(k_node_bwd<Node80>, P, a.n_atoms, s) : launch_tiles<Node64>(k_node_bwd<Node64>, P, a.n_atoms, s);
+}
+
+extern "C" int nb200_node_stall_probe(int64_t* prof, int32_t max_ctas) {
+    if (prof && max_ctas <= 0) return NB200_EINVAL;
+    g_prof = reinterpret_cast<long long*>(prof);
+    g_prof_ctas = prof ? max_ctas : 0;
+    return NB200_OK;
+}
diff --git a/nabladft_b200/csrc/tc_pipe.cuh b/nabladft_b200/csrc/tc_pipe.cuh
--- a/nabladft_b200/csrc/tc_pipe.cuh
+++ b/nabladft_b200/csrc/tc_pipe.cuh
@@ -11,9 +11,10 @@
 constexpr int WST_BYTES = 2 * (KSTAGE / 4) * WLBO;
 constexpr int STAGES_PER_TILE = 128 / KSTAGE;
 constexpr int WTILE_BYTES = STAGES_PER_TILE * WST_BYTES;
-template <bool TWO_GROUPS, int NT_ = 64>
+template <bool TWO_GROUPS, int NT_ = 64, bool PROBE_ = false>
 struct Layout {
     static constexpr bool two_groups = TWO_GROUPS;
+    static constexpr bool probe = PROBE_;
     static constexpr int NT = NT_;
     static constexpr int NEPI = TWO_GROUPS ? NWORK / 2 : NWORK, NLOAD = TWO_GROUPS ? NWORK / 2 : NWORK;
     static constexpr int CPT = NT / (NEPI / 4);
@@ -63,6 +64,9 @@
 };
 
 __device__ __forceinline__ void work_barrier() { asm volatile("bar.sync 1, %0;" ::"n"(32 * NWORK) : "memory"); }
+
+enum { PR_FULL, PR_XREADY, PR_STAGE_FREE, PR_MMA, PR_ISSUER, PR_XFREE, PR_ACC_FULL, PR_EPI, PR_BARRIER, PR_WORKER, NPROF };
+constexpr int PR_ROW = 16;
 __device__ __forceinline__ float4 ld4(const float* p) { return *reinterpret_cast<const float4*>(p); }
 
 template <class L>
@@ -74,7 +78,30 @@
     uint64_t *x_ready2, *x_free2;
     int xg = 0;
     int o = 0;
+    unsigned prof[L::probe ? NPROF : 1];
 };
+
+template <class L>
+__device__ __forceinline__ long long pclock() {
+    if constexpr (L::probe) return clock64();
+    else return 0;
+}
+template <class L>
+__device__ __forceinline__ void pspan(Ctx<L>& c, int k, long long t0) {
+    if constexpr (L::probe) c.prof[k] += (unsigned)(clock64() - t0);
+}
+template <class L>
+__device__ __forceinline__ void work_barrier(Ctx<L>& c) {
+    const long long t0 = pclock<L>();
+    work_barrier();
+    pspan(c, PR_BARRIER, t0);
+}
+template <class L>
+__device__ __forceinline__ void probe_store(const Ctx<L>& c, long long* row, int k0, int k1) {
+    if constexpr (L::probe) {
+        for (int k = k0; k < k1; ++k) atomicAdd(reinterpret_cast<unsigned long long*>(row) + k, (unsigned long long)c.prof[k]);
+    }
+}
 
 template <class L, class FlagFn, class TileFn>
 __device__ __forceinline__ void run_issuer_t(Ctx<L>& c, int n_units, FlagFn flags_of, TileFn tile_of, const unsigned char* wt, int spt = STAGES_PER_TILE) {
@@ -85,6 +112,7 @@
     const int n_q = n_units * spt;
     const bool leader = threadIdx.x == 32 * WARP_ISSUE;
     int q = 0, pending = -1;
+    const long long t_run = pclock<L>();
     auto release = [&](uint64_t* bar) { if (lane == 0) mbar_arrive(bar); };
     auto copy = [&](int qq) {
         if (!leader || qq >= n_q) return;
@@ -102,7 +130,7 @@
     for (int u = 0; u < n_units; ++u) {
         const int fl = flags_of(u);
         const bool newx = (fl & U_NEWX) != 0;
-        if (newx) { mbar_wait(c.x_ready, (uint32_t)(c.xg & 1)); ++c.xg; }
+        if (newx) { const long long t0 = pclock<L>(); mbar_wait(c.x_ready, (uint32_t)(c.xg & 1)); ++c.xg; pspan(c, PR_XREADY, t0); }
         if (fl & U_FIRST) {
 #pragma unroll
             for (int i = 0; i < NT / 2; ++i) { corr[i] = 0.f; main0[i] = 0.f; main1[i] = 0.f; }
@@ -112,7 +140,10 @@
             const int slot = q % W_STAGES;
             if (L::two_groups && newx && st == STAGES_PER_TILE / 2)
                 mbar_wait(c.x_ready2, (uint32_t)((c.xg - 1) & 1));
+            long long t0 = pclock<L>();
             mbar_wait(c.full + slot, (uint32_t)((q / W_STAGES) & 1));
+            pspan(c, PR_FULL, t0);
+            t0 = pclock<L>();
             const uint32_t wh = s_u32(c.ring + slot * WST_BYTES), wlo = wh + (KSTAGE / 4) * WLBO;
             const uint32_t xoff = (uint32_t)(st * (KSTAGE / 4) * XLBO);
             wgmma_fence();
@@ -127,6 +158,7 @@
             }
             wgmma_commit();
             wgmma_wait<1>();
+            pspan(c, PR_MMA, t0);
             if (pending >= 0) free_stage(pending);
             pending = q;
             if (L::two_groups && (fl & U_XLAST) && st == STAGES_PER_TILE / 2 - 1) {
@@ -135,14 +167,22 @@
                 release(c.x_free);
             }
         }
-        wgmma_wait<0>();
+        {
+            const long long t0 = pclock<L>();
+            wgmma_wait<0>();
+            pspan(c, PR_MMA, t0);
+        }
         if (pending >= 0) { free_stage(pending); pending = -1; }
         if (fl & U_XLAST) {
             if (!L::two_groups) release(c.x_free);
             else { if (spt < STAGES_PER_TILE / 2) release(c.x_free); release(c.x_free2); }
         }
         if (fl & U_LAST) {
-            if (c.o > 0) mbar_wait(c.stage_free, (uint32_t)((c.o - 1) & 1));
+            if (c.o > 0) {
+                const long long t0 = pclock<L>();
+                mbar_wait(c.stage_free, (uint32_t)((c.o - 1) & 1));
+                pspan(c, PR_STAGE_FREE, t0);
+            }
             const int f = 64 * h + 16 * wl + (lane >> 2);
 #pragma unroll
             for (int j = 0; j < NT / 8; ++j) {
@@ -154,13 +194,14 @@
             ++c.o;
         }
     }
+    pspan(c, PR_ISSUER, t_run);
 }
 template <class L>
 __device__ __forceinline__ void run_issuer(Ctx<L>& c, const Prog& prog, const unsigned char* wt) {
     run_issuer_t(c, prog.n, [&](int u) { return (int)prog.flag[u]; }, [&](int u) { return (int)prog.tile[u]; }, wt);
 }
 
-template <class L, class Fn>
+template <int RB_ = 0, class L, class Fn>
 __device__ __forceinline__ void load_x(Ctx<L>& c, int wtid, Fn f) {
     constexpr int NLOAD = L::NLOAD, NT = L::NT, XLBOF = L::XLBOF;
     if constexpr (L::two_groups) {
@@ -171,7 +212,11 @@
         float4 t[ITEMS];
 #pragma unroll
         for (int it = 0; it < ITEMS; ++it) t[it] = f(2 * (w8 + (NLOAD / 2) * it) + rsub, kc);
-        if (c.xg > 0) mbar_wait(half ? c.x_free2 : c.x_free, (uint32_t)((c.xg - 1) & 1));
+        if (c.xg > 0) {
+            const long long t0 = pclock<L>();
+            mbar_wait(half ? c.x_free2 : c.x_free, (uint32_t)((c.xg - 1) & 1));
+            pspan(c, PR_XFREE, t0);
+        }
 #pragma unroll
         for (int it = 0; it < ITEMS; ++it) {
             const int r = 2 * (w8 + (NLOAD / 2) * it) + rsub;
@@ -185,7 +230,7 @@
         ++c.xg;
         return;
     }
-    constexpr int RB = L::RPT % 8 == 0 ? 8 : L::RPT / 2;
+    constexpr int RB = RB_ > 0 ? RB_ : L::RPT % 8 == 0 ? 8 : L::RPT / 2;
     static_assert(L::RPT % RB == 0, "load_x one-group mapping");
     const int kc = wtid & 31, w = wtid >> 5;
 #pragma unroll 1
@@ -193,7 +238,11 @@
         float4 t[RB];
 #pragma unroll
         for (int it = 0; it < RB; ++it) t[it] = f(w + NLOAD * (RB * h + it), kc);
-        if (c.xg > 0) mbar_wait(c.x_free, (uint32_t)((c.xg - 1) & 1));
+        if (c.xg > 0) {
+            const long long t0 = pclock<L>();
+            mbar_wait(c.x_free, (uint32_t)((c.xg - 1) & 1));
+            pspan(c, PR_XFREE, t0);
+        }
 #pragma unroll
         for (int it = 0; it < RB; ++it) {
             const int r = w + NLOAD * (RB * h + it);
@@ -212,9 +261,13 @@
 struct XPut {
     float *hi, *lo;
     bool second;
-    __device__ __forceinline__ XPut(const Ctx<L>& c, int k) {
+    __device__ __forceinline__ XPut(Ctx<L>& c, int k) {
         second = L::two_groups && k >= 64;
-        if (c.xg > 0) mbar_wait(second ? c.x_free2 : c.x_free, (uint32_t)((c.xg - 1) & 1));
+        if (c.xg > 0) {
+            const long long t0 = pclock<L>();
+            mbar_wait(second ? c.x_free2 : c.x_free, (uint32_t)((c.xg - 1) & 1));
+            pspan(c, PR_XFREE, t0);
+        }
         hi = c.x_hi + (k >> 2) * L::XLBOF + (k & 3);
         lo = c.x_lo + (k >> 2) * L::XLBOF + (k & 3);
     }
@@ -232,19 +285,28 @@
 };
 
 template <class L>
-__device__ __forceinline__ void drain(Ctx<L>& c, int warp, int add_stage = 0) {
+__device__ __forceinline__ void stage_release(Ctx<L>& c) {
+    if (c.o > 0) mbar_arrive(c.stage_free);
+}
+
+template <class L>
+__device__ __forceinline__ void drain(Ctx<L>& c, int warp, int add_stage = 0, bool released = false) {
     float* mine = c.stage + (32 * (warp & 3) + (threadIdx.x & 31)) * L::SROW + (warp >> 2) * L::CPT;
     if (add_stage) {
         float4 keep[L::CPT / 4];
 #pragma unroll
         for (int i = 0; i < L::CPT / 4; ++i) keep[i] = reinterpret_cast<const float4*>(mine)[i];
-        if (c.o > 0) mbar_arrive(c.stage_free);
+        if (!released) stage_release(c);
+        const long long t0 = pclock<L>();
         mbar_wait(c.acc_full, (uint32_t)(c.o & 1));
+        pspan(c, PR_ACC_FULL, t0);
 #pragma unroll
         for (int i = 0; i < L::CPT / 4; ++i) reinterpret_cast<float4*>(mine)[i] = reinterpret_cast<const float4*>(mine)[i] + keep[i];
     } else {
-        if (c.o > 0) mbar_arrive(c.stage_free);
+        if (!released) stage_release(c);
+        const long long t0 = pclock<L>();
         mbar_wait(c.acc_full, (uint32_t)(c.o & 1));
+        pspan(c, PR_ACC_FULL, t0);
     }
     ++c.o;
 }
@@ -268,6 +330,7 @@
 template <class L>
 __device__ __forceinline__ Ctx<L> setup(unsigned char* smem, int tid) {
     Ctx<L> c;
+    if constexpr (L::probe) for (int k = 0; k < NPROF; ++k) c.prof[k] = 0;
     c.x_hi = reinterpret_cast<float*>(smem);
     c.x_lo = reinterpret_cast<float*>(smem + L::X_BYTES);
     c.ring = smem + 2 * L::X_BYTES;
@@ -292,14 +355,16 @@
 }
 
 template <class L, class Body>
-__device__ __forceinline__ void epi_chunks(const Ctx<L>& c, int warp, Body body) {
+__device__ __forceinline__ void epi_chunks(Ctx<L>& c, int warp, Body body) {
+    const long long t0 = pclock<L>();
 #pragma unroll 1
     for (int cb = 0; cb < L::CPT / L::CW; ++cb) {
         float v[L::CW];
         stage_ld(c, warp, L::CW * cb, v);
         body(cb, v);
     }
-}
-
-
-}
+    pspan(c, PR_EPI, t0);
+}
+
+
+}
```

New measurement: 72860 (median of 6 runs). 1.7% higher.
